# bo1929/krepp

Measured on AMD Instinct MI355X. Metric: reads/sec for `krepp dist` (150 bp), higher is better.
Workload: dtype u32/u64 integer + f64 likelihood; 1 GPU; 150bp reads vs 1000-genome synthetic index (Yule tree, -k 29 -w 35 -h 13, m4r1-frac, 2^25 rows), table inflated with random filler to 10 GB resident in HBM; index_inflated_in=a child process (handed over through /dev/shm), read_len=150, distinct_batches=2, lanes_per_batch=1, pipeline_streams=1, index_device_bytes=18867976828, hdist_th=4, parallelism=reads sharded x1, index replicated (RCCL bcast at load)

## Files before the change

### include/krepp_amd.h

```cpp
#ifndef KREPP_AMD_H
#define KREPP_AMD_H

#include <stddef.h>
#include <stdint.h>

#ifdef __cplusplus
extern "C" {
#endif

#define KR_API __attribute__((visibility("default")))

typedef enum kr_status {
  KR_OK = 0,
  KR_ERR_ARG = -1,
  KR_ERR_IO = -2,
  KR_ERR_FORMAT = -3,
  KR_ERR_NO_DEVICE = -4,
  KR_ERR_NOMEM = -5,
  KR_ERR_CAPACITY = -6,
  KR_ERR_STATE = -7,
  KR_ERR_UNSUPPORTED = -8
} kr_status;

#define KR_MAX_HDIST_TH 16u

typedef struct kr_host_index kr_host_index;

typedef struct kr_lib_view {
  const uint64_t* inc;
  const uint32_t* cmer;
  const uint32_t* pse;
  const double* rho;
  uint64_t nkmers;
  uint32_t nrows;
  uint32_t nsubsets;
  uint32_t nnodes;
  uint32_t r;
  uint32_t frac;
  uint32_t w;
} kr_lib_view;

typedef struct kr_index_view {
  uint32_t k, h, m;
  const uint8_t* ppos;
  const uint8_t* npos;
  uint32_t nlibs;
  const kr_lib_view* libs;
  uint32_t tree_nnodes;
  const uint8_t* node_kind;
  uint32_t wbackbone;
} kr_index_view;

KR_API int kr_host_index_load(const char* index_dir, kr_host_index** out);
KR_API int kr_host_sketch_load(const char* sketch_path, kr_host_index** out);
KR_API void kr_host_index_free(kr_host_index*);
KR_API int kr_host_index_view(const kr_host_index*, kr_index_view* out);
KR_API const char* kr_host_index_node_name(const kr_host_index*, uint32_t se);
KR_API const char* kr_host_index_node_label(const kr_host_index*, uint32_t se);
KR_API uint32_t kr_host_index_node_parent(const kr_host_index*, uint32_t se);
KR_API double kr_host_index_node_blen(const kr_host_index*, uint32_t se);

typedef struct kr_index kr_index;

#define KR_VIEW_HOST 0u
#define KR_VIEW_DEVICE 1u

KR_API int kr_index_upload(const kr_index_view* view, int device, uint32_t flags, kr_index** out);
KR_API void kr_index_free(kr_index*);

typedef struct kr_index_buffer {
  void* dptr;
  uint64_t bytes;
} kr_index_buffer;
KR_API int kr_index_export(const kr_index*, void* desc, uint64_t* desc_bytes, kr_index_buffer* bufs, uint32_t* nbufs);
KR_API int kr_index_import(const void* desc, uint64_t desc_bytes, int device, kr_index** out, kr_index_buffer* bufs,
                           uint32_t* nbufs);
KR_API uint64_t kr_index_device_bytes(const kr_index*);
KR_API uint32_t kr_index_slot_words(const kr_index*);
KR_API uint32_t kr_index_slot_format(const kr_index*);

KR_API int kr_index_broadcast(const kr_index* root, int ndev, const int* devices, kr_index** replicas);

typedef struct kr_params {
  uint32_t hdist_th;
  uint32_t tau;
  double chisq;
  double dist_max;
  uint32_t multi;
  uint32_t no_filter;
} kr_params;

KR_API void kr_params_default(kr_params*);

typedef struct kr_stream kr_stream;

KR_API int kr_stream_create(const kr_index*, const kr_params*, uint32_t max_reads, uint64_t max_bases,
                            uint64_t max_records, kr_stream** out);
KR_API void kr_stream_destroy(kr_stream*);

#define KR_BASES_HOST 0u
#define KR_BASES_DEVICE 1u
#define KR_TAP_ACCS 2u
#define KR_TAP_HITS 4u
#define KR_BASES_PINNED 8u
#define KR_ROWS_ONLY 16u
#define KR_ROWS_INDEXED 32u
#define KR_TILE_DEVICE 64u
#define KR_TILE_ROWS 128u

KR_API int kr_batch_submit(kr_stream*, const uint8_t* bases, const uint64_t* offsets, uint32_t nreads,
                           uint32_t flags);
KR_API int kr_batch_wait(kr_stream*);

typedef struct kr_result_view {
  uint32_t nreads;
  uint32_t nrecs;
  const uint32_t* read_off;
  const uint32_t* read_cnt;
  const uint32_t* read_onmers;
  const uint8_t* read_na;
  const uint32_t* rec_key;
  const uint8_t* rec_sel;
  const double* rec_d;
  const double* rec_v;
  const double* rec_chisq;
  const uint32_t* rec_hist;
  uint64_t rec_hist_stride;
  uint64_t nrows;
  const uint32_t* rec_dix;
  const double* dist_list;
  uint64_t ndist;
} kr_result_view;

KR_API int kr_batch_collect(kr_stream*, kr_result_view* out);
KR_API int kr_batch_collect_device(kr_stream*, kr_result_view* out);
KR_API int kr_debug_last_d2h_bytes(kr_stream*, uint64_t* bytes);
KR_API int kr_debug_place_fixed5(double v, char* out);

typedef struct kr_hit {
  uint32_t read;
  uint32_t kpos;
  uint32_t strand;
  uint32_t lib;
  uint64_t cmer_index;
  uint32_t hd;
  uint32_t se;
} kr_hit;
KR_API int kr_batch_hits(kr_stream*, const kr_hit** hits, uint64_t* nhits);
typedef struct kr_readtap {
  uint32_t hdist_filt[2];
} kr_readtap;
KR_API int kr_batch_readtaps(kr_stream*, const kr_readtap** taps);

KR_API int kr_debug_stream_move(kr_stream*, int which);
KR_API int kr_debug_stream_addrs(kr_stream*, uint64_t* out8);

KR_API int kr_debug_item_placement(kr_stream*, uint32_t* tried, uint32_t* kept, double* best_ns_per_read);

KR_API int kr_debug_front_end(const kr_index*, const uint8_t* bases, const uint64_t* offsets, uint32_t nreads,
                              uint32_t stride, uint32_t* rix, uint32_t* enc32, uint8_t* valid, uint8_t* pass);

KR_API int kr_debug_colour_classes(const uint32_t* pse_pairs , uint32_t nsubsets, const uint8_t* node_kind, uint32_t tree_nnodes,
                                   uint32_t* cls_out , uint32_t* pse_out , uint32_t* lists_out, uint64_t* nlist);

KR_API int kr_debug_brent(const kr_index*, uint32_t hdist_th, uint32_t n, const uint32_t* hist ,
                          const uint32_t* onmers, const double* rho, double* d_out, double* v_out);

KR_API int kr_debug_prefix(const uint32_t* values, uint32_t n, uint32_t block, uint32_t width, uint64_t* prefix , uint64_t* total);

KR_API int kr_llh_batch(const kr_index*, uint32_t hdist_th, uint32_t mode, uint64_t n, const double* hist, const double* uc,
                        const double* rho, const double* d_in, double* d_out, double* v_out);
KR_API int kr_llh_eval_indexed(const kr_index*, uint32_t th, uint64_t nprob, const double* hist, const double* uc, const double* rho,
                               uint64_t n, const uint32_t* pidx, const double* d_in, double* v_out);

typedef struct kr_timing {
  float ms_total;
  float ms_scan;
  float ms_acc;
  float ms_llh;
  float ms_h2d;
  uint32_t overflow_reads;
  uint32_t stack_spills;
  uint32_t lanes;
} kr_timing;
KR_API int kr_batch_timing(kr_stream*, kr_timing* out);

typedef struct kr_fastx kr_fastx;
typedef struct kr_fastx_batch {
  const uint8_t* bases;
  const uint64_t* offsets;
  const char* const* names;
  uint32_t nreads;
  uint32_t more;
} kr_fastx_batch;
KR_API int kr_fastx_open(const char* path, kr_fastx** out);
KR_API int kr_fastx_open_at(const char* path, uint64_t offset, kr_fastx** out);
KR_API int kr_fastx_next(kr_fastx*, uint64_t min_bases, kr_fastx_batch* out);
typedef struct kr_fastx_held kr_fastx_held;
KR_API int kr_fastx_detach(kr_fastx*, kr_fastx_held** out);
KR_API void kr_fastx_release(kr_fastx*, kr_fastx_held*);
KR_API uint64_t kr_fastx_parallel_chunks(const kr_fastx*);
KR_API void kr_fastx_pgz_stats(const kr_fastx*, uint64_t* parsed, uint64_t* discarded, uint64_t* gaps);
KR_API void kr_fastx_close(kr_fastx*);

KR_API int kr_format_dist(const kr_host_index*, const kr_result_view*, const char* const* names, char** text,
                          uint64_t* len);
KR_API int kr_format_seek(const kr_host_index*, const kr_index*, const kr_result_view*, uint32_t hdist_th,
                          const char* const* names, char** text, uint64_t* len);
KR_API int kr_stream_text_enable(kr_stream*, const kr_host_index*, uint64_t max_text_bytes, uint64_t max_id_bytes);
KR_API int kr_batch_submit_text(kr_stream*, const uint8_t* bases, const uint64_t* offsets, uint32_t nreads, uint32_t flags,
                                const char* ids, const uint32_t* id_off, uint32_t id_sep);
KR_API int kr_batch_collect_text(kr_stream*, const char** text, uint64_t* len);
KR_API uint32_t kr_debug_fixed5(double v, char* out);
KR_API void kr_free(void*);
KR_API void* kr_host_alloc(uint64_t bytes);
KR_API void kr_host_free(void*);

#define KR_FASTQ_OK 0u
#define KR_FASTQ_NOT_CLEAN 1u
#define KR_FASTQ_INCOMPLETE 2u
#define KR_FASTQ_LONG 3u
#define KR_FASTQ_CAPACITY 4u
typedef struct kr_fastq_parse {
  uint64_t consumed;
  uint64_t nbases;
  uint64_t id_bytes;
  uint64_t newlines;
  uint32_t nreads;
  uint32_t status;
  uint32_t rejected;
  uint32_t at_eof;
// ... 70 lines not shown
```

### krepp_amd/capi.py

```python
from __future__ import annotations

import ctypes as C
import os
from pathlib import Path

import numpy as np

_HERE = Path(__file__).resolve().parent
LIB_PATH = _HERE / "lib" / "libkrepp_amd.so"

KR_OK = 0
KR_ERR_ARG, KR_ERR_IO, KR_ERR_FORMAT, KR_ERR_NO_DEVICE = -1, -2, -3, -4
KR_ERR_NOMEM, KR_ERR_CAPACITY, KR_ERR_STATE, KR_ERR_UNSUPPORTED = -5, -6, -7, -8
KR_VIEW_HOST, KR_VIEW_DEVICE = 0, 1
KR_BASES_HOST, KR_BASES_DEVICE, KR_TAP_ACCS, KR_TAP_HITS, KR_BASES_PINNED, KR_ROWS_ONLY, KR_ROWS_INDEXED = 0, 1, 2, 4, 8, 16, 32
KR_TILE_DEVICE = 64
KR_TILE_ROWS = 128

u8p = C.POINTER(C.c_uint8)
u32p = C.POINTER(C.c_uint32)
u64p = C.POINTER(C.c_uint64)
f64p = C.POINTER(C.c_double)


class KrLibView(C.Structure):
    _fields_ = [("inc", u64p), ("cmer", u32p), ("pse", u32p), ("rho", f64p),
                ("nkmers", C.c_uint64), ("nrows", C.c_uint32), ("nsubsets", C.c_uint32),
                ("nnodes", C.c_uint32), ("r", C.c_uint32), ("frac", C.c_uint32), ("w", C.c_uint32)]


class KrIndexView(C.Structure):
    _fields_ = [("k", C.c_uint32), ("h", C.c_uint32), ("m", C.c_uint32),
                ("ppos", u8p), ("npos", u8p), ("nlibs", C.c_uint32), ("libs", C.POINTER(KrLibView)),
                ("tree_nnodes", C.c_uint32), ("node_kind", u8p), ("wbackbone", C.c_uint32)]


class KrIndexBuffer(C.Structure):
    _fields_ = [("dptr", C.c_void_p), ("bytes", C.c_uint64)]


class KrParams(C.Structure):
    _fields_ = [("hdist_th", C.c_uint32), ("tau", C.c_uint32), ("chisq", C.c_double),
                ("dist_max", C.c_double), ("multi", C.c_uint32), ("no_filter", C.c_uint32)]


class KrResultView(C.Structure):
    _fields_ = [("nreads", C.c_uint32), ("nrecs", C.c_uint32),
                ("read_off", u32p), ("read_cnt", u32p), ("read_onmers", u32p), ("read_na", u8p),
                ("rec_key", u32p), ("rec_sel", u8p), ("rec_d", f64p), ("rec_v", f64p),
                ("rec_chisq", f64p), ("rec_hist", u32p), ("rec_hist_stride", C.c_uint64), ("nrows", C.c_uint64),
                ("rec_dix", u32p), ("dist_list", f64p), ("ndist", C.c_uint64)]


class KrHit(C.Structure):
    _fields_ = [("read", C.c_uint32), ("kpos", C.c_uint32), ("strand", C.c_uint32), ("lib", C.c_uint32),
                ("cmer_index", C.c_uint64), ("hd", C.c_uint32), ("se", C.c_uint32)]


class KrTiming(C.Structure):
    _fields_ = [("ms_total", C.c_float), ("ms_scan", C.c_float), ("ms_acc", C.c_float), ("ms_llh", C.c_float),
                ("ms_h2d", C.c_float), ("overflow_reads", C.c_uint32), ("stack_spills", C.c_uint32), ("lanes", C.c_uint32)]


class KrFastxBatch(C.Structure):
    _fields_ = [("bases", u8p), ("offsets", u64p), ("names", C.POINTER(C.c_char_p)),
                ("nreads", C.c_uint32), ("more", C.c_uint32)]


KR_FASTQ_OK, KR_FASTQ_NOT_CLEAN, KR_FASTQ_INCOMPLETE, KR_FASTQ_LONG, KR_FASTQ_CAPACITY = 0, 1, 2, 3, 4


class KrFastqParse(C.Structure):
    _fields_ = [("consumed", C.c_uint64), ("nbases", C.c_uint64), ("id_bytes", C.c_uint64), ("newlines", C.c_uint64),
                ("nreads", C.c_uint32), ("status", C.c_uint32), ("rejected", C.c_uint32), ("at_eof", C.c_uint32),
                ("reserved", C.c_uint32 * 4)]


class KrMinimizerResult(C.Structure):
    _fields_ = [("keys", u64p), ("nkeys", C.c_uint64), ("n1", C.c_double), ("n2", C.c_double)]


class KrBuildParams(C.Structure):
    _fields_ = [("k", C.c_uint32), ("w", C.c_uint32), ("h", C.c_uint32), ("m", C.c_uint32), ("r", C.c_uint32),
                ("frac", C.c_uint32), ("num_threads", C.c_uint32), ("seed", C.c_uint32), ("ppos", u8p),
                ("gpu_minimizers", C.c_uint32), ("device", C.c_int32)]


EXPORTS = [
    "kr_host_index_load", "kr_host_sketch_load", "kr_format_seek", "kr_build_sketch", "kr_host_index_free", "kr_host_index_view", "kr_host_index_node_name",
    "kr_host_index_node_label", "kr_host_index_node_parent", "kr_host_index_node_blen",
    "kr_index_upload", "kr_index_free", "kr_index_export", "kr_index_import", "kr_index_device_bytes", "kr_index_slot_words", "kr_index_slot_format", "kr_index_broadcast",
    "kr_params_default", "kr_stream_create", "kr_stream_destroy", "kr_batch_submit", "kr_batch_wait",
    "kr_batch_collect", "kr_batch_collect_device", "kr_stream_text_enable", "kr_batch_submit_text", "kr_batch_collect_text",
    "kr_stream_fastq_enable", "kr_batch_submit_fastq", "kr_batch_fastq_names", "kr_debug_fastq_batch", "kr_debug_tile_layout", "kr_debug_tile_shape", "kr_batch_hits", "kr_batch_readtaps",
    "kr_debug_front_end", "kr_debug_stream_move", "kr_debug_stream_addrs", "kr_debug_item_placement", "kr_debug_brent", "kr_debug_prefix", "kr_debug_colour_classes", "kr_llh_batch", "kr_llh_eval_indexed", "kr_batch_timing",
    "kr_place_tree_create", "kr_place_tree_create_lineage", "kr_place_tree_nnodes", "kr_place_summary_add",
    "kr_place_summary_text", "kr_place_tree_free", "kr_place_tree_kinds", "kr_place_batch", "kr_place_stream", "kr_place_frame", "kr_place_counters",
    "kr_debug_last_d2h_bytes", "kr_debug_place_fixed5", "kr_place_text_counters", "kr_place_path_counters", "kr_fastx_open", "kr_fastx_open_at", "kr_fastx_next", "kr_fastx_detach", "kr_fastx_release", "kr_fastx_close", "kr_fastx_parallel_chunks", "kr_fastx_pgz_stats", "kr_format_dist", "kr_debug_fixed5", "kr_free", "kr_host_alloc", "kr_host_free",
    "kr_build_index", "kr_minimizers_cpu", "kr_minimizers_device", "kr_minimizers_free", "kr_last_error", "kr_version",
]

_lib = None


class KrError(RuntimeError):
    def __init__(self, code, msg):
        super().__init__(f"krepp_amd error {code}: {msg}")
        self.code = code


def load():
    global _lib
    if _lib is not None:
        return _lib
    if not LIB_PATH.exists():
        raise ImportError(f"{LIB_PATH} is missing: run `python -c 'import __graft_entry__ as g; g.build()'` "
                          "(the HIP extension is required; there is no CPU fallback)")
    lib = C.CDLL(str(LIB_PATH), mode=C.RTLD_GLOBAL)
    vp = C.c_void_p
    lib.kr_last_error.restype = C.c_char_p
    lib.kr_version.restype = C.c_char_p
    lib.kr_host_index_load.argtypes = [C.c_char_p, C.POINTER(vp)]
    lib.kr_host_index_free.argtypes = [vp]
    lib.kr_host_index_free.restype = None
    lib.kr_host_index_view.argtypes = [vp, C.POINTER(KrIndexView)]
    lib.kr_host_index_node_name.argtypes = [vp, C.c_uint32]
    lib.kr_host_index_node_name.restype = C.c_char_p
    lib.kr_host_index_node_label.argtypes = [vp, C.c_uint32]
    lib.kr_host_index_node_label.restype = C.c_char_p
    lib.kr_host_index_node_parent.argtypes = [vp, C.c_uint32]
    lib.kr_host_index_node_parent.restype = C.c_uint32
    lib.kr_host_index_node_blen.argtypes = [vp, C.c_uint32]
    lib.kr_host_index_node_blen.restype = C.c_double
    lib.kr_index_upload.argtypes = [C.POINTER(KrIndexView), C.c_int, C.c_uint32, C.POINTER(vp)]
    lib.kr_index_free.argtypes = [vp]
    lib.kr_index_free.restype = None
    lib.kr_index_export.argtypes = [vp, vp, u64p, C.POINTER(KrIndexBuffer), u32p]
    lib.kr_index_import.argtypes = [vp, C.c_uint64, C.c_int, C.POINTER(vp), C.POINTER(KrIndexBuffer), u32p]
    lib.kr_index_device_bytes.argtypes = [vp]
    lib.kr_index_broadcast.argtypes = [vp, C.c_int, C.POINTER(C.c_int), C.POINTER(vp)]
    lib.kr_index_device_bytes.restype = C.c_uint64
    lib.kr_index_slot_words.argtypes = [vp]
    lib.kr_index_slot_format.argtypes = [vp]
    lib.kr_index_slot_format.restype = C.c_uint32
    lib.kr_debug_stream_move.argtypes = [vp, C.c_int]
    lib.kr_debug_stream_addrs.argtypes = [vp, u64p]
    lib.kr_debug_item_placement.argtypes = [vp, u32p, u32p, C.POINTER(C.c_double)]
    lib.kr_index_slot_words.restype = C.c_uint32
    lib.kr_params_default.argtypes = [C.POINTER(KrParams)]
    lib.kr_params_default.restype = None
    lib.kr_stream_create.argtypes = [vp, C.POINTER(KrParams), C.c_uint32, C.c_uint64, C.c_uint64, C.POINTER(vp)]
    lib.kr_stream_destroy.argtypes = [vp]
    lib.kr_stream_destroy.restype = None
    lib.kr_batch_submit.argtypes = [vp, vp, vp, C.c_uint32, C.c_uint32]
    lib.kr_debug_fixed5.argtypes = [C.c_double, C.c_char_p]
    lib.kr_debug_fixed5.restype = C.c_uint32
    lib.kr_stream_text_enable.argtypes = [vp, vp, C.c_uint64, C.c_uint64]
    lib.kr_batch_submit_text.argtypes = [vp, vp, vp, C.c_uint32, C.c_uint32, vp, vp, C.c_uint32]
    lib.kr_batch_collect_text.argtypes = [vp, C.POINTER(vp), u64p]
    lib.kr_batch_wait.argtypes = [vp]
    lib.kr_batch_collect.argtypes = [vp, C.POINTER(KrResultView)]
    lib.kr_batch_collect_device.argtypes = [vp, C.POINTER(KrResultView)]
    lib.kr_batch_hits.argtypes = [vp, C.POINTER(C.POINTER(KrHit)), u64p]
    lib.kr_batch_readtaps.argtypes = [vp, C.POINTER(u32p)]
    lib.kr_debug_front_end.argtypes = [vp, vp, vp, C.c_uint32, C.c_uint32, vp, vp, vp, vp]
    lib.kr_debug_brent.argtypes = [vp, C.c_uint32, C.c_uint32, vp, vp, vp, vp, vp]
    lib.kr_debug_prefix.argtypes = [vp, C.c_uint32, C.c_uint32, C.c_uint32, vp, u64p]
    lib.kr_debug_colour_classes.argtypes = [vp, C.c_uint32, vp, C.c_uint32, vp, vp, vp, C.POINTER(C.c_uint64)]
    lib.kr_batch_timing.argtypes = [vp, C.POINTER(KrTiming)]
    lib.kr_llh_batch.argtypes = [vp, C.c_uint32, C.c_uint32, C.c_uint64, vp, vp, vp, vp, vp, vp]
    lib.kr_place_tree_create.argtypes = [vp, C.c_char_p, C.POINTER(vp)]
    lib.kr_place_tree_create_lineage.argtypes = [vp, C.c_char_p, C.POINTER(vp)]
    lib.kr_place_tree_nnodes.argtypes = [vp]
    lib.kr_place_tree_nnodes.restype = C.c_uint32
    lib.kr_place_summary_add.argtypes = [vp, vp, C.c_uint64, vp, C.POINTER(C.c_double)]
    lib.kr_place_summary_text.argtypes = [vp, vp, C.c_double, C.POINTER(vp), u64p]
    lib.kr_place_tree_free.argtypes = [vp]
    lib.kr_place_tree_free.restype = None
    lib.kr_place_tree_kinds.argtypes = [vp]
    lib.kr_place_tree_kinds.restype = u8p
    lib.kr_place_batch.argtypes = [vp, vp, vp, C.POINTER(KrResultView), vp, C.POINTER(C.c_char_p), C.POINTER(KrParams), C.c_int,
                                   C.POINTER(C.c_int), C.POINTER(vp), u64p, C.POINTER(vp), u64p]
    lib.kr_place_stream.argtypes = [vp, vp, vp, vp, C.c_uint32, vp, C.POINTER(C.c_char_p), C.POINTER(KrParams), C.c_int,
                                    C.POINTER(C.c_int), C.POINTER(vp), u64p, C.POINTER(vp), u64p]
    lib.kr_place_frame.argtypes = [vp, C.c_int, C.c_int, C.c_char_p, C.c_uint64, C.POINTER(vp), u64p]
    lib.kr_place_counters.argtypes = [u64p, u64p, u64p]
    lib.kr_place_counters.restype = None
    lib.kr_fastx_open.argtypes = [C.c_char_p, C.POINTER(vp)]
    lib.kr_fastx_open_at.argtypes = [C.c_char_p, C.c_uint64, C.POINTER(vp)]
    lib.kr_stream_fastq_enable.argtypes = [vp, C.c_uint64]
    lib.kr_batch_submit_fastq.argtypes = [vp, vp, C.c_uint64, C.c_uint32, C.c_uint32, C.POINTER(KrFastqParse)]
    lib.kr_batch_fastq_names.argtypes = [vp, C.POINTER(u64p), C.POINTER(u32p)]
    lib.kr_debug_fastq_batch.argtypes = [vp, vp, vp]
    lib.kr_debug_tile_layout.argtypes = [vp, u32p, u32p, vp, vp, vp, vp, vp]
    lib.kr_debug_tile_shape.argtypes = [C.c_uint64, C.c_uint32, u64p, u64p, u64p]
    lib.kr_fastx_next.argtypes = [vp, C.c_uint64, C.POINTER(KrFastxBatch)]
    lib.kr_fastx_detach.argtypes = [vp, C.POINTER(vp)]
    lib.kr_fastx_release.argtypes = [vp, vp]
    lib.kr_fastx_release.restype = None
    lib.kr_fastx_close.argtypes = [vp]
    lib.kr_fastx_close.restype = None
    lib.kr_format_dist.argtypes = [vp, C.POINTER(KrResultView), C.POINTER(C.c_char_p), C.POINTER(vp), u64p]
    lib.kr_free.argtypes = [vp]
    lib.kr_free.restype = None
    lib.kr_host_alloc.argtypes = [C.c_uint64]
    lib.kr_host_alloc.restype = vp
    lib.kr_host_free.argtypes = [vp]
    lib.kr_host_free.restype = None
    lib.kr_build_index.argtypes = [C.c_char_p, C.c_char_p, C.c_char_p, C.POINTER(KrBuildParams)]
    lib.kr_minimizers_cpu.argtypes = [C.POINTER(KrBuildParams), vp, vp, C.c_uint32, C.POINTER(KrMinimizerResult)]
    lib.kr_minimizers_device.argtypes = [C.c_int, C.POINTER(KrBuildParams), vp, vp, C.c_uint32, C.POINTER(KrMinimizerResult)]
    lib.kr_minimizers_free.argtypes = [C.POINTER(KrMinimizerResult)]
    lib.kr_minimizers_free.restype = None
    _lib = lib
    return lib


def check(rc):
    if rc != KR_OK:
        raise KrError(rc, load().kr_last_error().decode(errors="replace"))


def _np(ptr, n, dtype):
    if n == 0 or not ptr:
        return np.zeros(0, dtype=dtype)
    return np.ctypeslib.as_array(ptr, shape=(int(n),)).view(dtype).copy()

# ... 31 lines not shown
    def positions(self):
        return _np(self.view.ppos, self.view.h, np.uint8), _np(self.view.npos, self.view.k - self.view.h, np.uint8)

    def lib_arrays(self, i=0):
        lv = self.view.libs[i]
        return dict(inc=_np(lv.inc, lv.nrows, np.uint64), cmer=_np(lv.cmer, 2 * lv.nkmers, np.uint32).reshape(-1, 2),
                    pse=_np(lv.pse, 2 * lv.nsubsets, np.uint32).reshape(-1, 2), rho=_np(lv.rho, lv.nnodes, np.float64),
                    r=lv.r, frac=lv.frac, w=lv.w, nnodes=lv.nnodes, nsubsets=lv.nsubsets)

    def upload(self, device=0):
        return DeviceIndex.from_view(self.view, device, KR_VIEW_HOST, keep=self)

    def close(self):
        if self.h:
            self.lib.kr_host_index_free(self.h)
            self.h = C.c_void_p()

    def __del__(self):
        try:
            self.close()
        except Exception:
            pass


def default_params(**kw):
    p = KrParams()
    load().kr_params_default(C.byref(p))
    for k_, v in kw.items():
        setattr(p, k_, v)
    return p


class DeviceIndex:

    def __init__(self, handle, keep=None):
        self.lib = load()
        self.h = handle
        self._keep = keep

    @classmethod
    def from_view(cls, view, device=0, flags=KR_VIEW_HOST, keep=None):
        lib = load()
        h = C.c_void_p()
        check(lib.kr_index_upload(C.byref(view), int(device), int(flags), C.byref(h)))
        return cls(h, keep)

    def export(self):
        nb = C.c_uint64(0)
        n = C.c_uint32(0)
        check(self.lib.kr_index_export(self.h, None, C.byref(nb), None, C.byref(n)))
        desc = C.create_string_buffer(nb.value)
        bufs = (KrIndexBuffer * n.value)()
        check(self.lib.kr_index_export(self.h, desc, C.byref(nb), bufs, C.byref(n)))
        return desc.raw, [(b.dptr, b.bytes) for b in bufs]

    @classmethod
    def import_empty(cls, desc, device=0):
        lib = load()
        h = C.c_void_p()
        n = C.c_uint32(256)
        bufs = (KrIndexBuffer * 256)()
        check(lib.kr_index_import(desc, len(desc), int(device), C.byref(h), bufs, C.byref(n)))
        return cls(h), [(bufs[i].dptr, bufs[i].bytes) for i in range(n.value)]

    def broadcast(self, devices):
        n = len(devices)
        devs = (C.c_int * n)(*[int(d) for d in devices])
        outs = (C.c_void_p * n)()
        check(self.lib.kr_index_broadcast(self.h, n, devs, outs))
        return [DeviceIndex(C.c_void_p(outs[i])) for i in range(n)]

    @property
    def device_bytes(self):
        return int(self.lib.kr_index_device_bytes(self.h))

    @property
    def slot_words(self):
        return int(self.lib.kr_index_slot_words(self.h))

    @property
    def slot_format(self):
        return int(self.lib.kr_index_slot_format(self.h))

    def stream(self, params=None, max_reads=1 << 16, max_bases=None, max_records=0):
        return Stream(self, params or default_params(), max_reads, max_bases or max_reads * 160, max_records)

    def front_end(self, bases, offsets, stride):
        bases = np.ascontiguousarray(bases, dtype=np.uint8)
        offsets = np.ascontiguousarray(offsets, dtype=np.uint64)
        n = len(offsets) - 1
        rix = np.zeros((n, stride, 2), np.uint32)
        enc = np.zeros((n, stride, 2), np.uint32)
        valid = np.zeros((n, stride, 2), np.uint8)
        pas = np.zeros((n, stride, 2), np.uint8)
        check(self.lib.kr_debug_front_end(self.h, bases.ctypes.data, offsets.ctypes.data, n, stride,
                                          rix.ctypes.data, enc.ctypes.data, valid.ctypes.data, pas.ctypes.data))
        return rix, enc, valid, pas

    def brent(self, th, hist, onmers, rho):
        hist = np.ascontiguousarray(hist, dtype=np.uint32)
        onmers = np.ascontiguousarray(onmers, dtype=np.uint32)
        rho = np.ascontiguousarray(rho, dtype=np.float64)
        n = len(onmers)
        d = np.zeros(n)
        v = np.zeros(n)
        check(self.lib.kr_debug_brent(self.h, th, n, hist.ctypes.data, onmers.ctypes.data, rho.ctypes.data,
                                      d.ctypes.data, v.ctypes.data))
        return d, v

    def close(self):
        if self.h:
            self.lib.kr_index_free(self.h)
            self.h = C.c_void_p()

    def __del__(self):
        try:
            self.close()
        except Exception:
            pass


class Result:

    def __init__(self, rv, np_planes, copy_hist):
        n, c = rv.nreads, rv.nrecs
        self.nreads, self.nrecs, self.nrows = n, c, int(rv.nrows)
        self.read_off = _np(rv.read_off, n, np.uint32)
        self.read_cnt = _np(rv.read_cnt, n, np.uint32)
        self.read_onmers = _np(rv.read_onmers, n, np.uint32)
        self.read_na = _np(rv.read_na, n, np.uint8)
        key = _np(rv.rec_key, c, np.uint32)
        keep = key != 0
        self.rec_key = key[keep]
        self.rec_sel = _np(rv.rec_sel, c, np.uint8)[keep]
        if rv.rec_dix:
            self.rec_dix = _np(rv.rec_dix, c, np.uint32)[keep]
            self.dist_list = _np(rv.dist_list, int(rv.ndist), np.float64)
            self.rec_d = self.dist_list[self.rec_dix]
        else:
            self.rec_dix = None
            self.rec_d = _np(rv.rec_d, c, np.float64)[keep]
        self.rec_v = _np(rv.rec_v, c, np.float64)[keep] if rv.rec_v else None
        self.rec_chisq = _np(rv.rec_chisq, c, np.float64)[keep] if rv.rec_chisq else None
        self.rec_hist = (_np(rv.rec_hist, c * np_planes, np.uint32).reshape(np_planes, -1).T[keep]
                         if copy_hist and rv.rec_hist and c else (np.zeros((0, np_planes), np.uint32) if copy_hist else None))
        rr = np.zeros(c, np.uint32)
        nzr = np.nonzero(self.read_cnt)[0]
        if c and len(nzr):
            start = np.zeros(c, np.int64)
            start[self.read_off[nzr]] = self.read_off[nzr].astype(np.int64) + 1
            at = np.zeros(c + 1, np.uint32)
            at[self.read_off[nzr].astype(np.int64) + 1] = nzr
            rr = at[np.maximum.accumulate(start)]
        self.rec_read = rr[keep]
        newpos = np.cumsum(keep) - 1
        nz = self.read_cnt > 0
        self.read_off = np.where(nz, newpos[np.minimum(self.read_off, max(c - 1, 0))] if c else 0, 0).astype(np.uint32)
        self.nrecs = int(keep.sum())

    def rows(self):
        sel = self.rec_sel.astype(bool)
        return sorted(zip(self.rec_read[sel].tolist(), (self.rec_key[sel] >> 1).tolist(), self.rec_d[sel].tolist()))


class Stream:
    def __init__(self, dindex, params, max_reads, max_bases, max_records=0):
        self.lib = load()
        self.ix = dindex
        self.params = params
        self.h = C.c_void_p()
        check(self.lib.kr_stream_create(dindex.h, C.byref(params), int(max_reads), int(max_bases), int(max_records), C.byref(self.h)))
        self._keep = None
        self._flags = 0

    def submit(self, bases, offsets, flags=0):
        bases = np.ascontiguousarray(bases, dtype=np.uint8)
        offsets = np.ascontiguousarray(offsets, dtype=np.uint64)
        self._keep = (bases, offsets)
        self._flags = flags
        check(self.lib.kr_batch_submit(self.h, bases.ctypes.data, offsets.ctypes.data, len(offsets) - 1, flags))

    def submit_device(self, bases_ptr, offsets_ptr, nreads, flags=0):
        self._flags = flags | KR_BASES_DEVICE
        check(self.lib.kr_batch_submit(self.h, int(bases_ptr), int(offsets_ptr), int(nreads), self._flags))

    def wait(self):
        check(self.lib.kr_batch_wait(self.h))

    def collect(self):
        rv = KrResultView()
        check(self.lib.kr_batch_collect(self.h, C.byref(rv)))
        self._rv = rv
        return Result(rv, self.params.hdist_th + 1, bool(self._flags & KR_TAP_ACCS))

    def collect_view(self):
        rv = KrResultView()
        check(self.lib.kr_batch_collect(self.h, C.byref(rv)))
        self._rv = rv
        return rv

    def last_d2h_bytes(self):
        b = C.c_uint64(0)
        self.lib.kr_debug_last_d2h_bytes.argtypes = [C.c_void_p, C.POINTER(C.c_uint64)]
        check(self.lib.kr_debug_last_d2h_bytes(self.h, C.byref(b)))
        return int(b.value)

    def collect_device(self):
        rv = KrResultView()
        check(self.lib.kr_batch_collect_device(self.h, C.byref(rv)))
        return rv

    def hits(self):
        p = C.POINTER(KrHit)()
        n = C.c_uint64()
        check(self.lib.kr_batch_hits(self.h, C.byref(p), C.byref(n)))
        dt = np.dtype([("read", "<u4"), ("kpos", "<u4"), ("strand", "<u4"), ("lib", "<u4"), ("cmer_index", "<u8"),
                       ("hd", "<u4"), ("se", "<u4")])
        if n.value == 0:
            return np.zeros(0, dt)
        raw = C.string_at(p, n.value * C.sizeof(KrHit))
        return np.frombuffer(raw, dtype=dt).copy()

    def readtaps(self, nreads):
        p = u32p()
        check(self.lib.kr_batch_readtaps(self.h, C.byref(p)))
        return _np(p, 2 * nreads, np.uint32).reshape(-1, 2)

    def debug_move(self, which):
        check(self.lib.kr_debug_stream_move(self.h, which))

    def item_placement(self):
        a, b, c = C.c_uint32(0), C.c_uint32(0), C.c_double(0)
        check(self.lib.kr_debug_item_placement(self.h, C.byref(a), C.byref(b), C.byref(c)))
        return {"tried": a.value, "kept": b.value, "scan_ns_per_read": c.value}

    def debug_addrs(self):
        a = (C.c_uint64 * 8)()
        check(self.lib.kr_debug_stream_addrs(self.h, a))
        return dict(zip(("items", "counters", "cursors", "rd_off", "rd_it_off", "rd_filt", "rec_key", "dd"), [int(x) for x in a]))

    def timing(self):
        t = KrTiming()
        check(self.lib.kr_batch_timing(self.h, C.byref(t)))
        return t

    def format_seek(self, host_index, device_index, names, hdist_th=4):
        arr = (C.c_char_p * len(names))(*[n.encode() for n in names])
        txt = C.c_void_p()
        ln = C.c_uint64()
        self.lib.kr_format_seek.argtypes = [C.c_void_p, C.c_void_p, C.POINTER(KrResultView), C.c_uint32, C.POINTER(C.c_char_p),
                                            C.POINTER(C.c_void_p), C.POINTER(C.c_uint64)]
        check(self.lib.kr_format_seek(host_index.h, device_index.h, C.byref(self._rv), hdist_th, arr, C.byref(txt), C.byref(ln)))
        s = C.string_at(txt, ln.value).decode()
        self.lib.kr_free(txt)
        return s

    def text_enable(self, host_index, max_text_bytes, max_id_bytes):
        check(self.lib.kr_stream_text_enable(self.h, host_index.h, int(max_text_bytes), int(max_id_bytes)))
        self._text_on = True

    def submit_text(self, bases, offsets, names, flags=0, sep=1):
        bases = np.ascontiguousarray(bases, dtype=np.uint8)
        offsets = np.ascontiguousarray(offsets, dtype=np.uint64)
        enc = [n.encode() for n in names]
        blob = (b"\0" * sep).join(enc) + b"\0" * sep
        lens = np.fromiter((len(e) + sep for e in enc), dtype=np.uint32, count=len(enc))
        id_off = np.zeros(len(enc) + 1, dtype=np.uint32)
        np.cumsum(lens, out=id_off[1:])
        ids = np.frombuffer(blob, dtype=np.uint8)
        self._keep = (bases, offsets, ids, id_off)
        self._flags = flags | KR_ROWS_ONLY
        check(self.lib.kr_batch_submit_text(self.h, bases.ctypes.data, offsets.ctypes.data, len(offsets) - 1, flags, ids.ctypes.data, id_off.ctypes.data, sep))

    def submit_text_device(self, bases_ptr, offsets_ptr, nreads, names, flags=0, sep=1):
        enc = [n.encode() for n in names]
        ids = np.frombuffer((b"\0" * sep).join(enc) + b"\0" * sep, dtype=np.uint8)
        id_off = np.zeros(len(enc) + 1, dtype=np.uint32)
        np.cumsum(np.fromiter((len(e) + sep for e in enc), dtype=np.uint32, count=len(enc)), out=id_off[1:])
        self._keep = (ids, id_off)
        self._flags = flags | KR_BASES_DEVICE | KR_ROWS_ONLY
        check(self.lib.kr_batch_submit_text(self.h, int(bases_ptr), int(offsets_ptr), int(nreads), flags | KR_BASES_DEVICE, ids.ctypes.data, id_off.ctypes.data, sep))

    def fastq_enable(self, max_raw_bytes):
        check(self.lib.kr_stream_fastq_enable(self.h, int(max_raw_bytes)))

    def submit_fastq(self, raw, flags=0, at_eof=1):
        raw = bytes(raw)
        n = len(raw)
        if getattr(self, "_pinned_cap", 0) < max(n, 1):
            if getattr(self, "_pinned", None):
                self.lib.kr_host_free(self._pinned)
            self._pinned = self.lib.kr_host_alloc(max(n, 1))
            if not self._pinned:
                raise MemoryError("kr_host_alloc failed")
            self._pinned_cap = max(n, 1)
        C.memmove(self._pinned, raw, n)
        self._raw = raw
        out = KrFastqParse()
        check(self.lib.kr_batch_submit_fastq(self.h, self._pinned, n, flags, at_eof, C.byref(out)))
        self._fq_nreads = out.nreads
        text = getattr(self, "_text_on", False) and not (flags & (KR_TAP_ACCS | KR_TAP_HITS))
        self._flags = flags | KR_BASES_DEVICE | (KR_ROWS_ONLY if text else 0)
        return {f: getattr(out, f) for f in ("consumed", "nbases", "id_bytes", "newlines", "nreads", "status", "rejected", "at_eof")}

    def fastq_names(self):
        pos, ln = u64p(), u32p()
        check(self.lib.kr_batch_fastq_names(self.h, C.byref(pos), C.byref(ln)))
        n = self._fq_nreads
        if n == 0:
            return []
        p = np.ctypeslib.as_array(pos, shape=(n,))
        q = np.ctypeslib.as_array(ln, shape=(n,))
        return [self._raw[int(a):int(a) + int(b)].decode("latin-1") for a, b in zip(p, q)]

    def fastq_batch(self, summary):
        offs = np.zeros(summary["nreads"] + 1, np.uint64)
        bases = np.zeros(max(1, summary["nbases"]), np.uint8)
        check(self.lib.kr_debug_fastq_batch(self.h, bases.ctypes.data, offs.ctypes.data))
        return [bases[int(offs[i]):int(offs[i + 1])].tobytes() for i in range(summary["nreads"])]

    def tile_layout(self, nreads):
        nv, nl = C.c_uint32(0), C.c_uint32(0)
        check(self.lib.kr_debug_tile_layout(self.h, C.byref(nv), C.byref(nl), None, None, None, None, None))
        out = {"nv": int(nv.value), "nlong": int(nl.value)}
        if out["nv"] == 0:
            return out
        voff, vtile = np.zeros(out["nv"] + 1, np.uint64), np.zeros(out["nv"], np.uint8)
        rfirst, longs = np.zeros(nreads, np.uint32), np.zeros(2 * out["nlong"], np.uint32)
        check(self.lib.kr_debug_tile_layout(self.h, C.byref(nv), C.byref(nl), voff.ctypes.data, vtile.ctypes.data, rfirst.ctypes.data,
                                            longs.ctypes.data, None))
        bases = np.zeros(max(1, int(voff[-1])), np.uint8)
        check(self.lib.kr_debug_tile_layout(self.h, C.byref(nv), C.byref(nl), None, None, None, None, bases.ctypes.data))
        out.update(voff=voff, vtile=vtile, rfirst=rfirst, longs=longs.reshape(-1, 2), bases=bases[:int(voff[-1])])
        return out

    def collect_text(self):
        txt = C.c_void_p()
        ln = C.c_uint64()
        check(self.lib.kr_batch_collect_text(self.h, C.byref(txt), C.byref(ln)))
        return C.string_at(txt, ln.value) if ln.value else b""

    def format_dist(self, host_index, names):
        arr = (C.c_char_p * len(names))(*[n.encode() for n in names])
        txt = C.c_void_p()
        ln = C.c_uint64()
        check(self.lib.kr_format_dist(host_index.h, C.byref(self._rv), arr, C.byref(txt), C.byref(ln)))
        s = C.string_at(txt, ln.value).decode()
        self.lib.kr_free(txt)
        return s

    def close(self):
        if self.h:
            self.lib.kr_stream_destroy(self.h)
            self.h = C.c_void_p()
        if getattr(self, "_pinned", None):
            self.lib.kr_host_free(self._pinned)
            self._pinned, self._pinned_cap = None, 0

    def __del__(self):
        try:
            self.close()
        except Exception:
            pass


def tile_shape(length, k):
    a, b, c = C.c_uint64(0), C.c_uint64(0), C.c_uint64(0)
    check(load().kr_debug_tile_shape(int(length), int(k), C.byref(a), C.byref(b), C.byref(c)))
    return int(a.value), int(b.value), int(c.value)


def debug_prefix(values, block, width):
    values = np.ascontiguousarray(values, dtype=np.uint32)
    prefix = np.zeros(len(values), np.uint64)
    total = C.c_uint64(0)
    check(load().kr_debug_prefix(values.ctypes.data, len(values), block, width, prefix.ctypes.data, C.byref(total)))
    return prefix, total.value


def colour_classes(pse, node_kind):
    lib = load()
    pse = np.ascontiguousarray(pse, dtype=np.uint32).reshape(-1, 2)
    node_kind = np.ascontiguousarray(node_kind, dtype=np.uint8)
    n = len(pse)
    cls = np.zeros(n, np.uint32)
    out = np.zeros((n, 2), np.uint32)
    nl = C.c_uint64(0)
    rc = lib.kr_debug_colour_classes(pse.ctypes.data, n, node_kind.ctypes.data, len(node_kind) - 1, cls.ctypes.data, out.ctypes.data, None,
                                     C.byref(nl))
    lists = np.zeros(max(1, nl.value), np.uint32)
    if rc != 0:
        check(lib.kr_debug_colour_classes(pse.ctypes.data, n, node_kind.ctypes.data, len(node_kind) - 1, cls.ctypes.data, out.ctypes.data,
                                          lists.ctypes.data, C.byref(nl)))
    return cls, out, lists[: nl.value]


def read_fastx(path, min_bases=76800, stats=None, detach=0, offset=None):
    lib = load()
    lib.kr_fastx_parallel_chunks.restype = C.c_uint64
    lib.kr_fastx_parallel_chunks.argtypes = [C.c_void_p]
    h = C.c_void_p()
    if offset is None:
        check(lib.kr_fastx_open(os.fsencode(str(path)), C.byref(h)))
    else:
        check(lib.kr_fastx_open_at(os.fsencode(str(path)), int(offset), C.byref(h)))
    names, chunks, lens = [], [], []

    def take(b):
        if b.nreads:
            offs = np.ctypeslib.as_array(b.offsets, shape=(b.nreads + 1,)).copy()
            chunks.append(np.ctypeslib.as_array(b.bases, shape=(int(offs[-1]),)).copy() if offs[-1] else np.zeros(0, np.uint8))
            lens.extend(np.diff(offs).tolist())
            names.extend(b.names[i].decode() for i in range(b.nreads))

    held = []
    try:
        while True:
            b = KrFastxBatch()
            check(lib.kr_fastx_next(h, min_bases, C.byref(b)))
            if detach:
                hp = C.c_void_p()
                check(lib.kr_fastx_detach(h, C.byref(hp)))
                held.append((b, hp))
                while len(held) > detach:
                    ob, ohp = held.pop(0)
                    take(ob)
                    lib.kr_fastx_release(h, ohp)
            else:
                take(b)
            if not b.more:
                break
        for ob, ohp in held:
            take(ob)
            lib.kr_fastx_release(h, ohp)
    finally:
        if stats is not None:
            stats["parallel_chunks"] = int(lib.kr_fastx_parallel_chunks(h))
            a, b_, c_ = C.c_uint64(0), C.c_uint64(0), C.c_uint64(0)
            lib.kr_fastx_pgz_stats.restype = None
            lib.kr_fastx_pgz_stats.argtypes = [C.c_void_p, C.POINTER(C.c_uint64), C.POINTER(C.c_uint64), C.POINTER(C.c_uint64)]
            lib.kr_fastx_pgz_stats(h, C.byref(a), C.byref(b_), C.byref(c_))
            stats["gzip_chunks"] = {"parsed": int(a.value), "discarded": int(b_.value), "gaps": int(c_.value)}
        lib.kr_fastx_close(h)
    bases = np.concatenate(chunks) if chunks else np.zeros(0, np.uint8)
    offsets = np.zeros(len(lens) + 1, np.uint64)
    offsets[1:] = np.cumsum(np.asarray(lens, dtype=np.uint64))
    return names, bases, offsets


def place_counters():
    a, b = C.c_uint64(0), C.c_uint64(0)
    load().kr_place_counters(C.byref(a), C.byref(b), None)
    return int(a.value), int(b.value)


def place_text_counters():
    a, b = C.c_uint64(0), C.c_uint64(0)
    load().kr_place_text_counters.restype = None
    load().kr_place_text_counters(C.byref(a), C.byref(b))
    return int(a.value), int(b.value)
# ... 145 lines not shown
```

### krepp_amd/csrc/kr_common.h

```cpp
#ifndef KR_COMMON_H
#define KR_COMMON_H

#include "krepp_amd.h"

#include <atomic>
#include <cmath>
#include <cstdio>
#include <functional>
#include <string>
#include <vector>

namespace kr {

int fail(int code, const std::string& msg);
void clear_error();

struct TreeNode {
  std::string label;
  double blen;
  uint32_t parent;
  uint8_t kind;
};

struct HostTree {
  std::vector<TreeNode> nodes;
  uint32_t nnodes() const { return (uint32_t)nodes.size() - 1; }
  std::string name(uint32_t se) const;
};

bool parse_newick(const std::string& text, HostTree& out, std::string& err);
void balanced_tree(const std::vector<std::string>& names, HostTree& out);

void parallel_for(int n, const std::function<void(int)>& f);
int parallel_width();
unsigned usable_cpus();

uint64_t leaf_name_hash(const std::string& name);
uint64_t rehash64(uint64_t sh);

struct BuildCfg {
  uint32_t k, w, h, m, r;
  bool frac;
};
struct LshPositions {
  uint32_t k = 0, h = 0;
  std::vector<uint8_t> ppos, npos;
  std::vector<uint8_t> pasc;
  uint32_t rix(uint64_t bp) const;
  uint32_t enc32(uint64_t bp) const;
};
bool make_positions(uint32_t k, uint32_t h, const uint8_t* ppos, LshPositions& out);
double hll12_estimate(const uint8_t* reg);
inline int64_t build_row(uint32_t rix, const BuildCfg& c)
{
  uint32_t res = rix % c.m;
  if (c.frac ? res <= c.r : res == c.r) return c.frac ? (int64_t)(rix / c.m) * (c.r + 1) + res : (int64_t)(rix / c.m);
  return -1;
}
#if defined(__HIPCC__)
#define KR_HD __host__ __device__
#else
#define KR_HD
#endif
KR_HD inline bool fixed5_exact(double v, uint32_t* n_out)
{
  if (!(v >= 0.0 && v < 1000.0)) return false;
  const double sc = v * 100000.0;
  const double err = fma(v, 100000.0, -sc);
  const double fl = floor(sc), fr = sc - fl;
  uint32_t n = (uint32_t)fl;
  const double t = fr - 0.5;
  if (t > 0.0 || (t == 0.0 && (err > 0.0 || (err == 0.0 && (n & 1u))))) ++n;
  if (n >= 100000000u) return false;
  *n_out = n;
  return true;
}
KR_HD inline uint32_t fixed5_digits(uint32_t n, char* out)
{
  uint32_t ip = n / 100000u, fp = n - ip * 100000u;
  char tmp[4];
  uint32_t k = 0, o = 0;
  do {
    tmp[k++] = (char)('0' + ip % 10u);
    ip /= 10u;
  } while (ip);
  while (k) out[o++] = tmp[--k];
  out[o++] = '.';
  for (int q = 4; q >= 0; --q) {
    out[o + (uint32_t)q] = (char)('0' + fp % 10u);
    fp /= 10u;
  }
  return o + 5u;
}
inline size_t fmt_fixed5(double v, char* out)
{
  const bool neg = std::signbit(v);
  const double d = neg ? -v : v;
  if (d >= 0.0 && d < 1000.0) {
    const double sc = d * 100000.0, fl = std::floor(sc), fr = sc - fl;
    if (std::fabs(fr - 0.5) > 1e-6) {
      const uint64_t n = (uint64_t)fl + (fr > 0.5 ? 1u : 0u);
      uint64_t ip = n / 100000u, fp = n % 100000u;
      char tmp[8];
      size_t k = 0, o = 0;
      if (neg) out[o++] = '-';
      do {
        tmp[k++] = (char)('0' + ip % 10u);
        ip /= 10u;
      } while (ip);
      while (k) out[o++] = tmp[--k];
      out[o++] = '.';
      for (int q = 4; q >= 0; --q) {
        out[o + q] = (char)('0' + fp % 10u);
        fp /= 10u;
      }
      return o + 5;
    }
  }
  return (size_t)snprintf(out, 64, "%.5f", v);
}

inline uint64_t fmix64(uint64_t v)
{
  v ^= v >> 33;
  v *= 0xff51afd7ed558ccdull;
  v ^= v >> 33;
  v *= 0xc4ceb9fe1a85ec53ull;
  v ^= v >> 33;
  return v;
}
void extract_contig_cpu(const uint8_t* seq, uint64_t len, const BuildCfg& c, const LshPositions& lsh,
                        std::vector<uint64_t>& keys, double& n1, double& n2);
bool contig_end_special(const uint8_t* seq, uint64_t len, const BuildCfg& c, uint64_t& x, uint64_t& z);

struct PlaceTreeArrays {
  uint32_t pn = 0, nidx = 0;
  const uint32_t* parent = nullptr;
  const uint32_t* eff = nullptr;
  const uint8_t* elig = nullptr;
  const uint32_t* lo = nullptr;
  const uint32_t* idx_to_pt = nullptr;
  const uint32_t* depth = nullptr;
  const double* blen = nullptr;
  const uint32_t* card = nullptr;
  const char* labels = nullptr;
  const uint32_t* label_off = nullptr;
};
struct PlaceDeviceResult {
  uint32_t nreads = 0;
  const uint32_t* rd_c0 = nullptr;
  const uint32_t* rd_info = nullptr;
  const uint32_t* c_se = nullptr;
  const double *c_d = nullptr, *c_v = nullptr, *c_chisq = nullptr;
  uint64_t kept = 0;
  bool overflow = false;
  uint32_t heavy_reads = 0;
  const char* text = nullptr;
  uint64_t text_len = 0;
  uint64_t text_flags = 0;
};
}
struct kr_stream;
namespace kr {
int place_on_device(kr_stream* s, const void* tree_tag, const PlaceTreeArrays& T, const uint32_t* read_len, uint32_t tau,
                    bool no_filter, double chisq, PlaceDeviceResult* out);
int place_device_begin(kr_stream* s, const void* tree_tag, const PlaceTreeArrays& T, const uint32_t* read_len);
int place_device_launch(kr_stream* s, const PlaceTreeArrays& T, uint32_t r0, uint32_t n, uint32_t tau, bool no_filter, double chisq);
int place_device_finish(kr_stream* s, const PlaceTreeArrays& T, uint32_t r0, uint32_t n, uint32_t tau, bool no_filter, double chisq,
                        uint64_t kept_base, PlaceDeviceResult* out);
uint32_t place_stream_nreads(const kr_stream* s);
void* big_alloc(size_t n);
void big_free(void* p);
void place_device_abort(kr_stream* s);
int place_device_text_begin(kr_stream* s, const PlaceTreeArrays& T, const char* const* names, uint32_t nreads, int tabular, bool multi);
enum PlacePath : uint32_t {
  kPathRerunCand = 0, kPathRerunKeep, kPathListCut, kPathGivenUp, kPathText1, kPathText2, kPathText4, kPathText8, kPathText16, kPathRanges,
  kPathLastCnt0, kPathLastCnt3, kPathLastCnt12, kPathLastText, kPathLastCandCap, kPathLastKeepCap, kPathLastTextCap, kPathLastFlags,
  kPathLastTextFlags, kPathLastAttempts, kPathCount
};
extern std::atomic<uint64_t> g_place_paths[kPathCount];

}

#endif
```

### krepp_amd/csrc/kr_dev_common.inc

```

constexpr int kWave = 64;
constexpr int kSegPos = 128;
constexpr int kPlaneWords = kSegPos / 32;
constexpr int kMaxLibs = 16;
constexpr int kStackCap = 256;
constexpr int kLeanStack = 192;
__host__ __device__ inline uint32_t lean_stack_bytes(uint32_t bm_words) { uint32_t b = 5u * bm_words; b = (b + 15u) & ~15u; return b > kLeanStack * 8u ? b : kLeanStack * 8u; }
constexpr int kLdsSlots = 64;
#ifndef KR_ACC_LEAN_WPE
#define KR_ACC_LEAN_WPE 6
#endif
#ifndef KR_ACC_PIPE
#define KR_ACC_PIPE 1
#endif
#ifndef KR_ACC_LEAN_EV_WORDS
#define KR_ACC_LEAN_EV_WORDS 1216
#endif
#ifndef KR_ACC_LEAN2_EV_HALVES
#define KR_ACC_LEAN2_EV_HALVES 4
#endif
__host__ __device__ inline uint32_t lean_ev_words(uint32_t np, uint32_t segs = 1)
{
  const uint32_t w = KR_ACC_LEAN_EV_WORDS ? (uint32_t)KR_ACC_LEAN_EV_WORDS : (uint32_t)kLdsSlots * np * 5u ;
  return segs == 1 ? w : (w * (uint32_t)KR_ACC_LEAN2_EV_HALVES / 2u + 3u) & ~3u;
}
constexpr int kLdsProbeMax = 8;
constexpr int kMaxPlanes = KR_MAX_HDIST_TH + 1;
constexpr int kHistWords = (kMaxPlanes + 3) / 4;

constexpr uint32_t kSlotFilter = 9u;
__host__ __device__ inline uint32_t slot_words(uint32_t code) { return code == 0 ? 0u : (code == 8 ? 48u : (code == kSlotFilter ? 64u : 1u << code)); }

constexpr uint32_t kFiltLineCodes = 40u, kFiltSlotCodes = 80u;
constexpr uint32_t kFiltMaxTh = 6u;
__host__ __device__ inline uint32_t filt_code24(uint32_t enc) { return (enc & 0xFFFu) | ((enc >> 4) & 0xFFF000u); }
__host__ __device__ inline uint32_t filt_rest8(uint32_t enc) { return ((enc >> 12) & 0xFu) | ((enc >> 24) & 0xF0u); }

struct DevLib {
  const uint64_t* bkt;
  const uint32_t* enc;
  const uint32_t* se;
  const uint2* pse;
  const double* rho;
  const uint32_t* slots;
  const uint32_t* occ;
  const uint32_t* leaflist;
  const uint2* sx;
  uint64_t nkmers, nlist;
  uint32_t nrows, nsubsets, nnodes, numer;
  uint32_t slot_log2w;
};

struct DevIndex {
  uint32_t k, h, m, nlibs, tree_nnodes;
  uint32_t m_shift;
  PextMask pmask, nmask;
  const uint4* fe_tab;
  uint64_t ppk[2], npk[2];
  uint32_t nleaves;
  const uint32_t* node_info;
  const uint32_t* leaf_se;
  const int32_t* res_lib;
  const DevLib* libs;
  uint64_t res_mask;
  DevLib lib0;
};

struct LlhConst {
  uint32_t k, h, th, dbg;
  double binom_k[32];
  double binom_hnk[kMaxPlanes];
};

struct DevParams {
  uint32_t th, np;
  uint32_t multi, no_filter, dmax_set;
  uint32_t dbg;
  double chisq, dist_max;
};

enum CounterSlot : uint32_t {
  kCtRecSlots = 0,
  kCtErr = 1,
  kCtL2Reads = 2,
  kCtTapHits = 3,
  kCtRecords = 4,
  kCtLlhCursor = 5,
  kCtItemSlots = 6,
  kCtStEvents = 9,
  kCtStKeys = 10,
  kCtStBatches = 11,
  kCtStBig = 12,
  kCtStLevelTiles = 13,
  kCtStMaxKeys = 14,
  kCtStMaxEvents = 15,
  kCtCycLevel = 16,
  kCtCycFinalize = 17,
  kCtCycRead = 18,
  kCtProblems = 22,
  kCtLongReads = 25,
  kCtStackSpills = 26,
  kCtRows = 27,
  kCtTileHoles = 28,
  kCtCount = 29
};
constexpr uint32_t kCounterWords = (kCtCount + 31u) & ~31u;
enum CursorSet : uint32_t { kCurScan = 0, kCurAcc1 = 1 , kCurAccMerge = 2 , kCurAcc2 = 3 , kCurSets = 4 };

struct BatchOut {
  uint32_t* counters;
  uint32_t* cursors;
  uint32_t* rd_off;
  uint32_t* rd_cnt;
  uint32_t* rd_onmers;
  uint32_t* rd_filt;
  uint8_t* rd_na;
  uint32_t* rec_read;
  uint32_t* rec_key;
  uint32_t* rec_hist;
  double* rec_d;
  double* rec_v;
  double* rec_chisq;
  uint8_t* rec_sel;
  uint64_t* rec_w0;
  uint32_t hist_always;
  uint32_t keep_v;
  uint32_t* rec_rep;
  uint32_t* rep_list;
  double2* rep_dv;
  uint32_t rep_cap;
  ulonglong2* dd_table;
  uint32_t* dd_direct;
  double2* dd_dv;
  uint32_t* dd_ohist;
  uint8_t* dd_oslot;
  const uint8_t* dd_cls;
  uint32_t dd_nodes;
  uint32_t dd_slots;
  uint32_t dd_shift;
  uint32_t rec_cap;
  uint64_t rec_stride;
  kr_hit* hits;
  uint32_t hit_cap;
  uint2* items;
  const uint8_t* v_tile;
  uint32_t rows_mode;
  uint32_t* rd_rcnt;
  uint32_t* rd_roff;
  uint32_t* row_bsum;
  uint32_t* row_key;
  double* row_d;
  uint32_t rows_indexed;
  uint32_t* row_dix;
  double* dist_list;
  uint32_t item_cap;
  uint32_t* rd_it_off;
  uint32_t* rd_it_cnt;
  uint32_t rec_chunk;
  uint32_t* long_list;
  uint32_t* g_planes;
  uint32_t* g_counts;
  uint32_t* g_list;
  uint64_t* stk_spill;
  uint32_t nslots2;
  uint32_t g_list_words;
  uint32_t ev_spill, tab_spill, kt_spill;
  uint32_t bm_words;
};

enum : uint32_t { kErrRecCap = 1u, kErrStack = 2u, kErrTable = 4u, kErrHitCap = 8u, kErrItemCap = 16u };

// ... 298 lines not shown
```

### krepp_amd/csrc/kr_dev_likelihood.inc

```

struct LlhProblem {
  double mc[kMaxPlanes];
  double uc, rho;
};

struct DD {
  double hi, lo;
};
__device__ __forceinline__ DD dd_mul(DD a, DD b)
{
  double p = a.hi * b.hi;
  double e = fma(a.hi, b.hi, -p);
  e = fma(a.hi, b.lo, e);
  e = fma(a.lo, b.hi, e);
  double s = p + e;
  return DD{s, e - (s - p)};
}
__device__ __forceinline__ double pown_dd(double x, uint32_t n)
{
  DD r{1.0, 0.0}, b{x, 0.0};
  while (n) {
    if (n & 1u) r = dd_mul(r, b);
    n >>= 1;
    if (n) b = dd_mul(b, b);
// ... 1126 lines not shown
      tot += c[q];
    }
    uint32_t run = out.row_bsum[b] + block_scan_excl(tot);
#pragma unroll
    for (uint32_t q = 0; q < 4; ++q) {
      s_off[q0 + q] = run;
      if (rb + q0 + q < nreads) out.rd_roff[rb + q0 + q] = run;
      run += c[q];
    }
    __syncthreads();
    constexpr uint32_t U = 4;
    for (uint32_t qa = w; qa < kRowBlock && rb + qa < nreads; qa += 4u * U) {
      uint32_t o[U], n[U], ky[U], xr[U];
      double xd[U];
      uint8_t sl[U];
#pragma unroll
      for (uint32_t u = 0; u < U; ++u) {
        const uint32_t q = qa + 4u * u;
        const bool there = q < kRowBlock && rb + q < nreads;
        o[u] = there ? out.rd_off[rb + q] : 0u, n[u] = there ? out.rd_cnt[rb + q] : 0u;
      }
#pragma unroll
      for (uint32_t u = 0; u < U; ++u) {
        const bool on = lane < n[u];
        sl[u] = on ? out.rec_sel[o[u] + lane] : (uint8_t)0;
        ky[u] = on ? out.rec_key[o[u] + lane] : 0u;
        xr[u] = 0u, xd[u] = 0.0;
        if (INDEXED)
          xr[u] = on ? out.rec_rep[o[u] + lane] : 0u;
        else
          xd[u] = on ? out.rec_d[o[u] + lane] : 0.0;
      }
#pragma unroll
      for (uint32_t u = 0; u < U; ++u) {
        const uint32_t q = qa + 4u * u;
        if (n[u] == 0) continue;
        uint32_t pos = s_off[q];
        {
          const bool sel = sl[u] != 0;
          const uint64_t sm = __ballot(sel);
          if (sel) {
            const uint32_t at = pos + (uint32_t)__popcll(sm & lt);
            out.row_key[at] = ky[u];
            if (INDEXED)
              out.row_dix[at] = xr[u];
            else
              out.row_d[at] = xd[u];
          }
          pos += (uint32_t)__popcll(sm);
        }
        for (uint32_t i0 = 64u; i0 < n[u]; i0 += 64u) {
          const uint32_t i = i0 + lane;
          const bool sel = i < n[u] && out.rec_sel[o[u] + i] != 0;
          const uint64_t sm = __ballot(sel);
          if (sel) {
            const uint32_t at = pos + (uint32_t)__popcll(sm & lt);
            out.row_key[at] = out.rec_key[o[u] + i];
            if (INDEXED)
              out.row_dix[at] = out.rec_rep[o[u] + i];
            else
              out.row_d[at] = out.rec_d[o[u] + i];
          }
          pos += (uint32_t)__popcll(sm);
        }
      }
    }
    __syncthreads();
  }
}

__global__ void kr_build_occ(const uint64_t* bkt, uint32_t nrows, uint32_t* occ)
{
  const uint32_t nw = (nrows + 31u) / 32u;
  for (uint32_t w = blockIdx.x * blockDim.x + threadIdx.x; w < nw; w += gridDim.x * blockDim.x) {
    uint32_t bits = 0;
    for (uint32_t j = 0; j < 32u; ++j) {
      const uint32_t r = w * 32u + j;
      if (r < nrows && (bkt[r] & 0xFFFFFFull) != 0) bits |= 1u << j;
    }
    occ[w] = bits;
  }
}

__global__ void kr_build_slots(const uint64_t* bkt, const uint32_t* enc, uint32_t nrows, uint32_t words, uint32_t* slots)
{
  const uint64_t n = (uint64_t)nrows * words;
  for (uint64_t i = blockIdx.x * (uint64_t)blockDim.x + threadIdx.x; i < n; i += (uint64_t)gridDim.x * blockDim.x) {
    const uint32_t row = (uint32_t)(i / words), wd = (uint32_t)(i - (uint64_t)row * words);
    const uint64_t b = bkt[row];
    const uint64_t st = b >> 24;
    const uint32_t ln = (uint32_t)(b & 0xFFFFFFu);
    uint32_t x = 0xFFFFFFFFu;
    if (wd == 0)
      x = ln;
    else if (wd == 1)
      x = (uint32_t)st;
    else if (wd - 2u < ln)
      x = enc[st + wd - 2u];
    slots[i] = x;
  }
}
```

### krepp_amd/csrc/kr_dev_scan.inc

```

constexpr int kListCap = 128;
struct ProbeList {
  lds_u64* bkt;
  lds_u32* q;
  lds_u32* tag;
};

struct Cand {
  uint64_t b0, b1;
  uint32_t q0, q1;
  uint32_t lib0, lib1;
};

template <bool SL, bool SLOT>
__device__ __forceinline__ Cand fetch_group_fe(const DevIndex& ix, const FrontEnd& fe, uint32_t& nvalid)
{
  Cand c;
  nvalid = __popcll(__ballot(fe.valid));
  int lib = -1;
  c.b0 = 0, c.b1 = 0, c.lib0 = 0, c.lib1 = 0;
  c.q0 = fe.enc32[0];
  c.q1 = fe.enc32[1];
  const uint32_t* d0 = nullptr;
  const uint32_t* d1 = nullptr;
// ... 64 lines not shown
  uint32_t rd_start;
  uint32_t err;
  uint32_t filt0, filt1;
  uint32_t cur_seg;
  uint32_t n_st;
  lds_u64* stage;
};
constexpr uint32_t kItemStage = 256;
#ifndef KR_ITEM_CHUNK
#define KR_ITEM_CHUNK 2048
#endif
constexpr uint32_t kItemChunk = KR_ITEM_CHUNK;
#ifndef KR_SCAN_READ_CHUNK
#define KR_SCAN_READ_CHUNK 32
#endif
constexpr uint32_t kReadChunk = KR_SCAN_READ_CHUNK;
constexpr uint32_t kCursors = 32, kCursorStride = 32;
struct ReadCursor {
  uint32_t* cur;
  uint32_t nreads, range, c, tried, chunk;
  __device__ __forceinline__ void init(uint32_t* base, uint32_t n, uint32_t home, uint32_t reads_per_visit = kReadChunk)
  {
    cur = base, nreads = n, range = (n + kCursors - 1) / kCursors, c = home % kCursors, tried = n ? 0 : kCursors, chunk = reads_per_visit;
  }
  __device__ __forceinline__ bool next(uint32_t& r0, uint32_t& r1)
  {
    while (tried < kCursors) {
      const uint32_t lo = c * range, hi = min(lo + range, nreads);
      uint32_t o = 0;
      if (lane_id() == 0) o = atomicAdd(&cur[c * kCursorStride], chunk);
      o = __shfl(o, 0);
      if (lo + o < hi) {
        r0 = lo + o, r1 = min(r0 + chunk, hi);
        return true;
      }
      c = (c + 1) % kCursors, ++tried;
    }
    return false;
  }
};

__device__ __forceinline__ bool item_reserve(const BatchOut& out, ScanWave& sw, uint32_t n)
{
  if (sw.it_next + n <= sw.it_end) return true;
  const uint32_t have = sw.it_next - sw.rd_start;
  const uint32_t size = (have + n + kItemChunk + 15u) & ~15u;
  uint32_t base = 0;
  if (lane_id() == 0) base = atomicAdd(&out.counters[kCtItemSlots], size);
  base = __shfl(base, 0);
  if ((uint64_t)base + size > out.item_cap) {
    sw.err |= kErrItemCap;
    return false;
  }
  if (have) {
    __builtin_amdgcn_fence(__ATOMIC_ACQ_REL, "workgroup");
    for (uint32_t i = lane_id(); i < have; i += 64) {
      const uint32_t* src = reinterpret_cast<const uint32_t*>(out.items + sw.rd_start + i);
      out.items[base + i] = make_uint2(gload(src), gload(src + 1));
    }
  }
  sw.rd_start = base;
  sw.it_next = base + have;
  sw.it_end = base + size;
  return true;
}

__device__ __forceinline__ void flush_stage(const BatchOut& out, ScanWave& sw)
{
  if (sw.n_st == 0) return;
  WAVE_SYNC();
  const uint32_t n16 = (sw.n_st + 15u) & ~15u;
  if (item_reserve(out, sw, n16)) {
    for (uint32_t i = lane_id(); i < n16; i += 64) {
      const uint64_t v = i < sw.n_st ? sw.stage[i] : 0ull;
      out.items[sw.it_next + i] = make_uint2((uint32_t)v, (uint32_t)(v >> 32));
    }
    sw.it_next += sw.n_st;
  }
  sw.n_st = 0;
  WAVE_SYNC();
}

constexpr uint32_t kItemMarker = 0x80000000u;
template <bool SL, bool TAP, bool FK = false>
__device__ __forceinline__ void emit_hits(const DevIndex& ix, const BatchOut& out, ScanWave& sw, uint32_t read, uint32_t base0,
                                          uint32_t tg, uint64_t e_al, uint32_t c, uint32_t pend, uint32_t hds)
{
  const uint64_t lt = (1ull << lane_id()) - 1ull;
  const uint32_t seg = base0 >> 7;
  while (__ballot(pend != 0) != 0) {
    const bool has = pend != 0;
    const uint32_t e = has ? (uint32_t)__ffs((int)pend) - 1u : 0u;
    const uint32_t hd = (hds >> (8u * e)) & 31u;
    const uint64_t idx = e_al + 4ull * c + e;
    if (has) {
      if (tag_strand(tg))
        sw.filt1 = min(sw.filt1, hd);
      else
        sw.filt0 = min(sw.filt0, hd);
      if (TAP) {
        const uint32_t se = get_lib<SL>(ix, tag_lib(tg)).se[idx];
        const uint32_t hix = atomicAdd(&out.counters[kCtTapHits], 1u);
        if (hix < out.hit_cap) {
          kr_hit h;
          h.read = read;
          h.kpos = base0 + tag_pos(tg);
          h.strand = tag_strand(tg);
          h.lib = tag_lib(tg);
          h.cmer_index = idx;
          h.hd = hd;
          h.se = (se >> 30) == 1u ? ix.leaf_se[se & kColMask] : (se & kColMask);
          out.hits[hix] = h;
        } else {
          atomicOr(&out.counters[kCtErr], kErrHitCap);
        }
      }
    }
    const uint64_t hm = __ballot(has);
    const uint32_t mark = seg != sw.cur_seg ? 1u : 0u;
    if (sw.n_st + (uint32_t)__popcll(hm) + mark > kItemStage) flush_stage(out, sw);
    if (mark && lane_id() == 0) sw.stage[sw.n_st] = (uint64_t)seg | ((uint64_t)kItemMarker << 32);
    sw.n_st += mark;
    sw.cur_seg = seg;
    if (has)
      sw.stage[sw.n_st + __popcll(hm & lt)] =
        (uint64_t)(uint32_t)idx | ((uint64_t)(FK ? ((tg & 0xFFFu) | (7u << 12) | (hd << 15) | ((uint32_t)(idx >> 32) << 23))
                                                 : ((tg & 0xFFFu) | (hd << 12) | ((uint32_t)(idx >> 32) << 17))) << 32);
    sw.n_st += (uint32_t)__popcll(hm);
    pend &= pend - 1u;
  }
}

template <int LOG_G, int CPL, bool SL, bool TAP>
__device__ __forceinline__ void scan_group(const DevIndex& ix, const DevParams& P, const BatchOut& out, ScanWave& sw,
                                           const ProbeList& pl, lds_u32* queue, lds_u32* stepinfo, uint32_t nact, uint32_t read,
                                           uint32_t base0)
{
  constexpr uint32_t G = 1u << LOG_G, PPS = 64u >> LOG_G;
  constexpr uint32_t kBits = 64u / CPL * CPL;
  const uint32_t lane = lane_id(), sub = lane & (G - 1u);
  uint32_t p0 = 0, cb = 0;
  while (p0 < nact) {
    uint64_t hitbits = 0;
    uint32_t step = 0;
    while (p0 < nact && step < kBits) {
      const uint32_t pi = p0 + (lane >> LOG_G);
      const bool on = pi < nact;
      const uint64_t b = on ? pl.bkt[pi] : 0ull;
      const uint32_t q = on ? pl.q[pi] : 0u;
      const uint64_t st = b >> 24;
      const uint32_t tot = (uint32_t)(st & 3u) + (uint32_t)(b & 0xFFFFFFu);
      const uint32_t nch = on ? (tot + 3u) >> 2 : 0u;
      const uint32_t* enc = get_lib<SL>(ix, SL ? 0u : tag_lib(pl.tag[on ? pi : 0u])).enc + (st & ~3ull);
      for (; step < kBits && __ballot(sub + cb * G < nch) != 0; cb += CPL, step += CPL) {
        if (lane < (uint32_t)CPL) stepinfo[step + lane] = p0 | (((cb + lane) * G) << 8);
        uint4 v[CPL];
#pragma unroll
        for (int j = 0; j < CPL; ++j) {
          const uint32_t c = sub + (cb + (uint32_t)j) * G;
          v[j] = make_uint4(0, 0, 0, 0);
          if (c < nch) v[j] = *reinterpret_cast<const uint4*>(enc + 4u * c);
        }
        uint32_t r = 0;
#pragma unroll
        for (int j = 0; j < CPL; ++j) {
          const uint32_t m = min(min(hd_lr32(v[j].x, q), hd_lr32(v[j].y, q)), min(hd_lr32(v[j].z, q), hd_lr32(v[j].w, q)));
          r |= (m <= P.th && sub + (cb + (uint32_t)j) * G < nch) ? (1u << j) : 0u;
        }
        hitbits |= (uint64_t)r << step;
      }
      if (__ballot(sub + cb * G < nch) == 0) p0 += PPS, cb = 0;
    }
    if (P.dbg & 1u) hitbits = 0;
    const uint32_t cnt = (uint32_t)__popcll(hitbits);
    uint32_t inc = cnt;
#pragma unroll
    for (int d = 1; d < 64; d <<= 1) {
      const uint32_t o = __shfl_up(inc, d);
      if (lane >= (uint32_t)d) inc += o;
    }
    const uint32_t H = __shfl(inc, 63);
    uint64_t hb = hitbits;
    uint32_t slot = inc - cnt;
    WAVE_SYNC();
    for (uint32_t w0 = 0; w0 < H; w0 += 64) {
      while (__ballot(hb != 0 && slot < w0 + 64u) != 0) {
        if (hb != 0 && slot < w0 + 64u) {
          const uint32_t si = stepinfo[(uint32_t)__ffsll((long long)hb) - 1u];
          queue[slot - w0] = ((si & 255u) + (lane >> LOG_G)) | ((sub + (si >> 8)) << 8);
          hb &= hb - 1;
          ++slot;
        }
      }
      WAVE_SYNC();
      uint32_t pend = 0, hds = 0, tg = 0, c = 0;
      uint64_t e_al = 0;
      if (lane < min(64u, H - w0)) {
        const uint32_t d = queue[lane], probe = d & 255u;
        c = d >> 8;
        const uint64_t b = pl.bkt[probe];
// ... 3 lines not shown
        e_al = st & ~3ull;
        const int rel0 = (int)(st & 3u), tot = rel0 + (int)(uint32_t)(b & 0xFFFFFFu);
        const uint4 v = *reinterpret_cast<const uint4*>(get_lib<SL>(ix, tag_lib(tg)).enc + e_al + 4u * c);
        pend = chunk_hits(v, rel0 - 4 * (int)c, tot - 4 * (int)c, q, P.th, hds);
      }
      WAVE_SYNC();
      emit_hits<SL, TAP>(ix, out, sw, read, base0, tg, e_al, c, pend, hds);
    }
  }
}

template <int LOG_G, int CPL, bool SL, bool TAP>
__device__ __forceinline__ void scan_group_slots(const DevIndex& ix, const DevParams& P, const BatchOut& out, ScanWave& sw,
                                                 const ProbeList& pl, lds_u32* queue, uint32_t nact, uint32_t read, uint32_t base0)
{
  constexpr uint32_t G = 1u << LOG_G, PPS = 64u >> LOG_G, W = G * CPL * 4u, CAP = W - 2u;
  static_assert((kListCap / PPS) * CPL <= 64, "one hit bit per (pass, chunk)");
  const uint32_t lane = lane_id(), sub = lane & (G - 1u);
  uint64_t hitbits = 0;
  uint32_t step = 0;
  for (uint32_t p0 = 0; p0 < nact; p0 += PPS, step += CPL) {
    const uint32_t pi = p0 + (lane >> LOG_G);
    const bool on = pi < nact;
    const uint32_t row = on ? (uint32_t)pl.bkt[pi] : 0u;
    const uint32_t q = on ? pl.q[pi] : 0u;
    const DevLib L = get_lib<SL>(ix, SL ? 0u : tag_lib(pl.tag[on ? pi : 0u]));
    const uint32_t* slot = L.slots + (uint64_t)row * W;
    uint4 v[CPL];
#pragma unroll
    for (int j = 0; j < CPL; ++j) {
      v[j] = make_uint4(0, 0, 0, 0);
      if (on) v[j] = *reinterpret_cast<const uint4*>(slot + 4u * (sub + (uint32_t)j * G));
    }
    uint32_t r = 0;
#pragma unroll
    for (int j = 0; j < CPL; ++j) {
      const uint32_t m = min(min(hd_lr32(v[j].x, q), hd_lr32(v[j].y, q)), min(hd_lr32(v[j].z, q), hd_lr32(v[j].w, q)));
      r |= (m <= P.th && on) ? (1u << j) : 0u;
    }
    hitbits |= (uint64_t)r << step;
    if (__ballot(on && sub == 0 && v[0].x > CAP) != 0) {
      const uint32_t blen = __shfl(v[0].x, lane & ~(G - 1u)), bstart = __shfl(v[0].y, lane & ~(G - 1u));
      const bool lg = on && blen > CAP;
      const uint64_t st = (uint64_t)bstart + CAP;
      const uint64_t e_al = st & ~3ull;
      const int rel0 = (int)(st & 3u), tot = rel0 + (lg ? (int)(blen - CAP) : 0);
      const uint32_t nch = lg ? (uint32_t)(tot + 3) >> 2 : 0u;
      const uint32_t tg = pl.tag[on ? pi : 0u];
      for (uint32_t c = sub; __ballot(c < nch) != 0; c += G) {
        uint32_t pend = 0, hds = 0;
        if (c < nch) {
          const uint4 w = *reinterpret_cast<const uint4*>(L.enc + e_al + 4u * c);
          pend = chunk_hits(w, rel0 - 4 * (int)c, tot - 4 * (int)c, q, P.th, hds);
        }
        if (P.dbg & 1u) pend = 0;
        emit_hits<SL, TAP>(ix, out, sw, read, base0, tg, e_al, c, pend, hds);
      }
    }
  }
  if (P.dbg & 1u) hitbits = 0;
  const uint32_t cnt = (uint32_t)__popcll(hitbits);
  uint32_t inc = cnt;
#pragma unroll
  for (int d = 1; d < 64; d <<= 1) {
    const uint32_t o = __shfl_up(inc, d);
    if (lane >= (uint32_t)d) inc += o;
  }
  const uint32_t H = __shfl(inc, 63);
  uint64_t hb = hitbits;
  uint32_t slot_i = inc - cnt;
  for (uint32_t w0 = 0; w0 < H; w0 += 64) {
    while (__ballot(hb != 0 && slot_i < w0 + 64u) != 0) {
      if (hb != 0 && slot_i < w0 + 64u) {
        const uint32_t bit = (uint32_t)__ffsll((long long)hb) - 1u;
        const uint32_t pass = bit / (uint32_t)CPL, j = bit - pass * (uint32_t)CPL;
        queue[slot_i - w0] = (pass * PPS + (lane >> LOG_G)) | ((sub + j * G) << 8);
        hb &= hb - 1;
        ++slot_i;
      }
    }
    WAVE_SYNC();
    uint32_t pend = 0, hds = 0, tg = 0, c = 0;
    uint64_t e_al = 0;
    if (lane < min(64u, H - w0)) {
      const uint32_t d = queue[lane], probe = d & 255u;
      c = d >> 8;
      const uint32_t row = (uint32_t)pl.bkt[probe];
      const uint32_t q = pl.q[probe];
      tg = pl.tag[probe];
      const uint32_t* slot = get_lib<SL>(ix, tag_lib(tg)).slots + (uint64_t)row * W;
      const uint2 hdr = *reinterpret_cast<const uint2*>(slot);
      const uint4 v = *reinterpret_cast<const uint4*>(slot + 4u * c);
      const int nin = (int)min(hdr.x, CAP);
      pend = chunk_hits(v, 2 - 4 * (int)c, nin + 2 - 4 * (int)c, q, P.th, hds);
      e_al = (uint64_t)hdr.y - 2ull;
    }
    WAVE_SYNC();
    emit_hits<SL, TAP>(ix, out, sw, read, base0, tg, e_al, c, pend, hds);
  }
}

template <int LOG_G, int CPL, bool SL, bool TAP, bool SLOT>
__device__ __forceinline__ void scan_read(const DevIndex& ix, const DevParams& P, const BatchIn& in, const BatchOut& out,
                                          uint32_t read, ScanWave& sw, const ProbeList& pl, lds_u32* queue, lds_u32* stepinfo, lds_u32* meta)
{
  const uint32_t lane = lane_id();
  const uint64_t lt = (1ull << lane) - 1ull;
  const uint64_t off0 = in.offsets[read], off1 = in.offsets[read + 1];
  const uint8_t* seq = in.bases + off0;
  const uint64_t len = off1 - off0;
  const uint32_t k = ix.k;
  const uint64_t nkm = len >= k ? len - k + 1 : 0;
  uint32_t onmers = 0;
  sw.it_next = min((sw.it_next + 15u) & ~15u, sw.it_end);
  sw.rd_start = sw.it_next;
  sw.n_st = 0;
  sw.cur_seg = 0;
  sw.filt0 = 0xFFFFFFFFu, sw.filt1 = 0xFFFFFFFFu;
  for (uint64_t base0 = 0; base0 < nkm; base0 += kSegPos) {
    const uint32_t npos_seg = (uint32_t)min((uint64_t)kSegPos, nkm - base0);
    SegBits sb;
    load_segment(seq, len, base0, sb);
#pragma unroll
    for (int pp = 0; pp < 2; ++pp) {
      if (pp == 1 && npos_seg <= 64) break;
      uint32_t nv = 0;
      const Cand cur = fetch_group<SL, SLOT>(ix, sb, pp, npos_seg, nv);
      onmers += nv;
      const bool a0 = SLOT ? cur.b0 != 0 : (cur.b0 & 0xFFFFFFu) != 0, a1 = SLOT ? cur.b1 != 0 : (cur.b1 & 0xFFFFFFu) != 0;
      const uint64_t m0 = __ballot(a0), m1 = __ballot(a1);
      const uint32_t n0 = __popcll(m0), nact = n0 + __popcll(m1);
      if (a0) {
        const uint32_t i = __popcll(m0 & lt);
        pl.bkt[i] = cur.b0;
        pl.q[i] = cur.q0;
        pl.tag[i] = (64u * pp + lane) | (cur.lib0 << 8);
      }
      if (a1) {
        const uint32_t i = n0 + __popcll(m1 & lt);
        pl.bkt[i] = cur.b1;
        pl.q[i] = cur.q1;
        pl.tag[i] = (64u * pp + lane) | (1u << 7) | (cur.lib1 << 8);
      }
      WAVE_SYNC();
      if (!(P.dbg & 4u)) {
        if (SLOT)
          scan_group_slots<LOG_G, CPL, SL, TAP>(ix, P, out, sw, pl, queue, nact, read, (uint32_t)base0);
        else
          scan_group<LOG_G, CPL, SL, TAP>(ix, P, out, sw, pl, queue, stepinfo, nact, read, (uint32_t)base0);
      }
      WAVE_SYNC();
    }
  }
  flush_stage(out, sw);
  uint32_t f0 = sw.filt0, f1 = sw.filt1;
#pragma unroll
  for (int d = 32; d >= 1; d >>= 1) {
    f0 = min(f0, (uint32_t)__shfl_xor(f0, d));
    f1 = min(f1, (uint32_t)__shfl_xor(f1, d));
  }
  if (lane == 0) {
    meta[0 * kReadChunk] = sw.rd_start;
    meta[1 * kReadChunk] = sw.it_next - sw.rd_start;
    meta[2 * kReadChunk] = onmers;
    meta[3 * kReadChunk] = f0;
    meta[4 * kReadChunk] = f1;
  }
}

#ifndef KR_SCAN_WPE
#define KR_SCAN_WPE 6
#endif
#ifndef KR_SCAN_WPE_SLOT
#define KR_SCAN_WPE_SLOT 4
#endif
constexpr int kScanWaves = 4;
template <int LOG_G, int CPL, bool SL, bool TAP, bool SLOT>
__global__ __launch_bounds__(kScanWaves* kWave, (SLOT ? KR_SCAN_WPE_SLOT : KR_SCAN_WPE)) void kr_scan_kernel_t(DevIndex ix, DevParams P, BatchIn in, BatchOut out)
{
  __shared__ __attribute__((aligned(16))) uint64_t s_bkt[kScanWaves][kListCap];
  __shared__ uint32_t s_q[kScanWaves][kListCap], s_tag[kScanWaves][kListCap], s_queue[kScanWaves][64], s_step[kScanWaves][64];
// ... 34 lines not shown
```

### krepp_amd/csrc/kr_dev_scan_pipe.inc

```

#ifndef KR_SCAN_DEPTH
#define KR_SCAN_DEPTH 1
#endif
#ifndef KR_SCAN_PIPE_WPE
#define KR_SCAN_PIPE_WPE 4
#endif
#ifndef KR_SCAN_PIPE_FE
#define KR_SCAN_PIPE_FE 2
#endif

struct SlotList {
  lds_u32* row;
  lds_u32* q;
  lds_u32* tag;
};
struct GroupDesc {
  uint32_t nact, read, base0, slot;
  bool last;
};

struct SegRaw {
  uint32_t c[3];
};
__device__ __forceinline__ SegRaw segment_request(const uint8_t* seq, uint64_t len, uint64_t base0)
// ... 124 lines not shown
#pragma unroll
  for (int d = 0; d < DEPTH; ++d) {
    const uint32_t pi = (c * DEPTH + (uint32_t)d) * PPS + (lane >> LOG_G);
    const bool on = pi < nact;
    const uint32_t row = on ? L.row[pi] : 0u;
    const uint32_t* slot = get_lib<SL>(ix, SL ? 0u : tag_lib(L.tag[on ? pi : 0u])).slots + (uint64_t)row * W;
#pragma unroll
    for (int j = 0; j < CPL; ++j) {
      v[d * CPL + j] = make_uint4(0, 0, 0, 0);
      if (on) v[d * CPL + j] = *reinterpret_cast<const uint4*>(slot + 4u * (sub + (uint32_t)j * G));
    }
  }
}

template <int LOG_G, int CPL, int DEPTH, bool SL, bool TAP>
__device__ __forceinline__ uint64_t pipe_test(const DevIndex& ix, const DevParams& P, const BatchOut& out, ScanWave& sw, const SlotList& L,
                                              const GroupDesc& g, uint32_t c, const uint4 (&v)[DEPTH * CPL])
{
  constexpr uint32_t G = 1u << LOG_G, PPS = 64u >> LOG_G, W = G * CPL * 4u, CAP = W - 2u;
  const uint32_t lane = lane_id(), sub = lane & (G - 1u);
  uint64_t bits = 0;
#pragma unroll
  for (int d = 0; d < DEPTH; ++d) {
    const uint32_t p = c * DEPTH + (uint32_t)d;
    const uint32_t pi = p * PPS + (lane >> LOG_G);
    const bool on = pi < g.nact;
    const uint32_t q = on ? L.q[pi] : 0u;
    uint32_t r = 0;
#pragma unroll
    for (int j = 0; j < CPL; ++j) {
      const uint4 w = v[d * CPL + j];
      const uint32_t m = min(min(hd_lr32(w.x, q), hd_lr32(w.y, q)), min(hd_lr32(w.z, q), hd_lr32(w.w, q)));
      r |= (m <= P.th && on) ? (1u << j) : 0u;
    }
    bits |= (uint64_t)r << (p * CPL);
    const uint32_t blen0 = v[d * CPL].x;
    if (__ballot(on && sub == 0 && blen0 > CAP) != 0) {
      const uint32_t blen = __shfl(blen0, lane & ~(G - 1u)), bstart = __shfl(v[d * CPL].y, lane & ~(G - 1u));
      const bool lg = on && blen > CAP;
      const uint64_t st = (uint64_t)bstart + CAP;
      const uint64_t e_al = st & ~3ull;
      const int rel0 = (int)(st & 3u), tot = rel0 + (lg ? (int)(blen - CAP) : 0);
      const uint32_t nch = lg ? (uint32_t)(tot + 3) >> 2 : 0u;
      const uint32_t tg = L.tag[on ? pi : 0u];
      const DevLib Lb = get_lib<SL>(ix, SL ? 0u : tag_lib(tg));
      for (uint32_t cc = sub; __ballot(cc < nch) != 0; cc += G) {
        uint32_t pend = 0, hds = 0;
        if (cc < nch) {
          const uint4 w = *reinterpret_cast<const uint4*>(Lb.enc + e_al + 4u * cc);
          pend = chunk_hits(w, rel0 - 4 * (int)cc, tot - 4 * (int)cc, q, P.th, hds);
        }
        if (P.dbg & 1u) pend = 0;
        emit_hits<SL, TAP>(ix, out, sw, g.read, g.base0, tg, e_al, cc, pend, hds);
      }
    }
  }
  return (P.dbg & 1u) ? 0ull : bits;
}

template <int LOG_G, int CPL, bool SL, bool TAP>
__device__ __forceinline__ void pipe_resolve(const DevIndex& ix, const DevParams& P, const BatchOut& out, ScanWave& sw, const SlotList& L,
                                             lds_u32* queue, const GroupDesc& g, uint64_t hitbits)
{
  constexpr uint32_t G = 1u << LOG_G, PPS = 64u >> LOG_G, W = G * CPL * 4u, CAP = W - 2u;
  const uint32_t lane = lane_id(), sub = lane & (G - 1u);
  const uint32_t cnt = (uint32_t)__popcll(hitbits);
  const uint32_t inc = wave_scan_incl(cnt);
  const uint32_t H = (uint32_t)__builtin_amdgcn_readlane((int)inc, 63);
  uint64_t hb = hitbits;
  uint32_t slot_i = inc - cnt;
  for (uint32_t w0 = 0; w0 < H; w0 += 64) {
    while (__ballot(hb != 0 && slot_i < w0 + 64u) != 0) {
      if (hb != 0 && slot_i < w0 + 64u) {
        const uint32_t bit = (uint32_t)__ffsll((long long)hb) - 1u;
        const uint32_t pass = bit / (uint32_t)CPL, j = bit - pass * (uint32_t)CPL;
        queue[slot_i - w0] = (pass * PPS + (lane >> LOG_G)) | ((sub + j * G) << 8);
        hb &= hb - 1;
        ++slot_i;
      }
    }
    WAVE_SYNC();
    uint32_t pend = 0, hds = 0, tg = 0, c = 0;
    uint64_t e_al = 0;
    if (lane < min(64u, H - w0)) {
      const uint32_t d = queue[lane], probe = d & 255u;
      c = d >> 8;
      const uint32_t row = L.row[probe];
      const uint32_t q = L.q[probe];
      tg = L.tag[probe];
      const uint32_t* slot = get_lib<SL>(ix, tag_lib(tg)).slots + (uint64_t)row * W;
      const uint2 hdr = *reinterpret_cast<const uint2*>(slot);
      const uint4 v = *reinterpret_cast<const uint4*>(slot + 4u * c);
      const int nin = (int)min(hdr.x, CAP);
      pend = chunk_hits(v, 2 - 4 * (int)c, nin + 2 - 4 * (int)c, q, P.th, hds);
      e_al = (uint64_t)hdr.y - 2ull;
    }
    WAVE_SYNC();
    emit_hits<SL, TAP>(ix, out, sw, g.read, g.base0, tg, e_al, c, pend, hds);
  }
}

__device__ __forceinline__ void pipe_begin_read(ScanWave& sw)
{
  sw.it_next = min((sw.it_next + 15u) & ~15u, sw.it_end);
  sw.rd_start = sw.it_next;
  sw.n_st = 0;
  sw.cur_seg = 0;
  sw.filt0 = 0xFFFFFFFFu, sw.filt1 = 0xFFFFFFFFu;
}
__device__ __forceinline__ void pipe_end_read(const BatchOut& out, ScanWave& sw, lds_u32* meta)
{
  flush_stage(out, sw);
  uint32_t f0 = sw.filt0, f1 = sw.filt1;
#pragma unroll
  for (int d = 32; d >= 1; d >>= 1) {
    f0 = min(f0, (uint32_t)__shfl_xor(f0, d));
    f1 = min(f1, (uint32_t)__shfl_xor(f1, d));
  }
  if (lane_id() == 0) {
    meta[0 * kReadChunk] = sw.rd_start;
    meta[1 * kReadChunk] = sw.it_next - sw.rd_start;
    meta[3 * kReadChunk] = f0;
    meta[4 * kReadChunk] = f1;
  }
}

template <int LOG_G, int CPL, int DEPTH, int WPE, bool SL, bool TAP>
__global__ __launch_bounds__(kScanWaves* kWave, WPE) void kr_scan_pipe_kernel_t(DevIndex ix, DevParams P, BatchIn in, BatchOut out)
{
  constexpr uint32_t PPS = 64u >> LOG_G;
  static_assert((kListCap / PPS) * CPL <= 64, "one hit bit per (pass, chunk)");
  __shared__ uint32_t s_row[kScanWaves][2][kListCap], s_q[kScanWaves][2][kListCap], s_tag[kScanWaves][2][kListCap], s_queue[kScanWaves][64];
  __shared__ uint32_t s_meta[kScanWaves][5 * kReadChunk];
  __shared__ __attribute__((aligned(16))) uint64_t s_stage[kScanWaves][kItemStage];
  __shared__ __attribute__((aligned(16))) uint4 s_fetab[KR_SCAN_PIPE_FE == 2 ? 1024 : 1];
  static_assert(kReadChunk <= 64, "one lane per read of a visit");
  if (KR_SCAN_PIPE_FE == 2) {
    fe_tab_to_lds(ix, (lds_u32x4*)s_fetab);
    __syncthreads();
  }
  const uint32_t w = threadIdx.x / kWave;
  SlotList LA{(lds_u32*)s_row[w][0], (lds_u32*)s_q[w][0], (lds_u32*)s_tag[w][0]};
  SlotList LB{(lds_u32*)s_row[w][1], (lds_u32*)s_q[w][1], (lds_u32*)s_tag[w][1]};
  lds_u32* queue = (lds_u32*)s_queue[w];
  lds_u32* meta = (lds_u32*)s_meta[w];
  ScanWave sw;
  sw.it_next = sw.it_end = sw.rd_start = 0;
  sw.err = 0;
  sw.cur_seg = 0;
  sw.n_st = 0;
  sw.stage = (lds_u64*)s_stage[w];
  sw.filt0 = sw.filt1 = 0xFFFFFFFFu;
  ReadCursor rc;
  rc.init(out.cursors + kCurScan * kCursors * kCursorStride, in.nreads, blockIdx.x * kScanWaves + w);
  uint32_t r0v, r1v;
  GroupGen<SL, KR_SCAN_PIPE_FE> gen;
  gen.tab = (const lds_u32x4*)s_fetab;
  uint4 v[DEPTH * CPL];
  while (rc.next(r0v, r1v)) {
    const uint32_t r0 = (uint32_t)__builtin_amdgcn_readfirstlane((int)r0v), r1 = (uint32_t)__builtin_amdgcn_readfirstlane((int)r1v);
    gen.init(r0, r1);
    GroupDesc ga, gb;
    bool flip = false;
    bool has_a = gen.next(ix, P, in, LA, meta, ga);
    if (has_a) {
      gen.prefetch(ix, in);
      pipe_begin_read(sw);
      pipe_issue<LOG_G, CPL, DEPTH, SL>(ix, LA, ga.nact, 0, v);
    }
    uint32_t c = 0;
    uint64_t hitbits = 0;
    bool has_b = false;
    while (has_a) {
      const SlotList& A = flip ? LB : LA;
      const SlotList& B = flip ? LA : LB;
      if (c == 0) {
        has_b = gen.next(ix, P, in, B, meta, gb);
        if (has_b) gen.prefetch(ix, in);
      }
      hitbits |= pipe_test<LOG_G, CPL, DEPTH, SL, TAP>(ix, P, out, sw, A, ga, c, v);
      const uint32_t npass = (ga.nact + PPS - 1u) / PPS;
// ... 27 lines not shown
```

### krepp_amd/csrc/kr_host_index.inc

```

struct kr_index {
  int device = 0;
  uint32_t log_g = 0;
  uint32_t slot_log2w = 0;
  DevIndex dix;
  std::vector<DevLib> hlibs;
  std::vector<void*> allocs;
  std::vector<kr_index_buffer> bufs;
  std::vector<uint8_t> desc;
  uint64_t bytes = 0;
  mutable std::mutex chain_mu;
  static constexpr uint32_t kChainEvents = 16;
  mutable hipEvent_t chain_ev[kChainEvents] = {nullptr};
  mutable uint32_t chain_n = 0;
  mutable bool chain_off = false;
  mutable std::mutex llh_mu;
  mutable DevBuf<double> llh_dev;
  mutable PinBuf<double> llh_pin;
  mutable DevBuf<char> d_names;
  mutable DevBuf<uint32_t> d_name_off;
};

namespace {

struct DescHeader {
  uint32_t magic, k, h, m, nlibs, tree_nnodes, nleaves, log_g;
  uint32_t slot_log2w, occ;
  uint64_t res_mask;
  uint8_t ppos[32], npos[32];
};
struct DescLib {
  uint64_t nkmers, nlist;
  uint32_t nrows, nsubsets, nnodes, numer;
};

int dev_alloc(kr_index* ix, void** p, uint64_t bytes)
{
  HIP_TRY(hipMalloc(p, bytes ? bytes : 16));
  ix->allocs.push_back(*p);
  ix->bytes += bytes;
  return KR_OK;
}

int alloc_from_desc(kr_index* ix, const DescHeader& H, const std::vector<DescLib>& L)
{
  ix->hlibs.resize(H.nlibs);
  ix->bufs.clear();
  for (uint32_t i = 0; i < H.nlibs; ++i) {
    DevLib& d = ix->hlibs[i];
    memset(&d, 0, sizeof(d));
    d.nkmers = L[i].nkmers, d.nlist = L[i].nlist, d.nrows = L[i].nrows, d.nsubsets = L[i].nsubsets, d.nnodes = L[i].nnodes,
    d.numer = L[i].numer;
    void* p;
    int rc;
    uint64_t b;
    b = (uint64_t)d.nrows * 8;
    if ((rc = dev_alloc(ix, &p, b))) return rc;
    d.bkt = (const uint64_t*)p;
    ix->bufs.push_back({p, b});
    b = (d.nkmers + 16) * 4;
    if ((rc = dev_alloc(ix, &p, b))) return rc;
    d.enc = (const uint32_t*)p;
    ix->bufs.push_back({p, b});
    b = (d.nkmers + 16) * 4;
    if ((rc = dev_alloc(ix, &p, b))) return rc;
    d.se = (const uint32_t*)p;
    ix->bufs.push_back({p, b});
    b = (uint64_t)d.nsubsets * 8;
    if ((rc = dev_alloc(ix, &p, b))) return rc;
    d.pse = (const uint2*)p;
    ix->bufs.push_back({p, b});
    b = (uint64_t)d.nnodes * 8;
    if ((rc = dev_alloc(ix, &p, b))) return rc;
    d.rho = (const double*)p;
    ix->bufs.push_back({p, b});
    b = d.nlist * 4;
    if ((rc = dev_alloc(ix, &p, b))) return rc;
    d.leaflist = (const uint32_t*)p;
    ix->bufs.push_back({p, b});
    if (H.occ) {
      b = (((uint64_t)d.nrows + 31) / 32) * 4;
      if ((rc = dev_alloc(ix, &p, b))) return rc;
      d.occ = (const uint32_t*)p;
      ix->bufs.push_back({p, b});
    }
    d.slot_log2w = H.slot_log2w;
    if (H.slot_log2w) {
      b = (uint64_t)d.nrows * slot_words(H.slot_log2w) * 4;
      if ((rc = dev_alloc(ix, &p, b))) return rc;
      d.slots = (const uint32_t*)p;
      ix->bufs.push_back({p, b});
    }
    if (H.slot_log2w == kSlotFilter) {
      b = (uint64_t)d.nrows * kFiltSlotCodes * 8;
      if ((rc = dev_alloc(ix, &p, b))) return rc;
      d.sx = (const uint2*)p;
      ix->bufs.push_back({p, b});
    }
  }
  void* p;
  int rc;
  uint64_t b = ((uint64_t)H.tree_nnodes + 1) * 4;
  if ((rc = dev_alloc(ix, &p, b))) return rc;
  ix->dix.node_info = (const uint32_t*)p;
  ix->bufs.push_back({p, b});
  b = (uint64_t)std::max<uint32_t>(1u, H.nleaves) * 4;
  if ((rc = dev_alloc(ix, &p, b))) return rc;
  ix->dix.leaf_se = (const uint32_t*)p;
  ix->bufs.push_back({p, b});
  ix->dix.nleaves = H.nleaves;
  ix->log_g = H.log_g;
  ix->slot_log2w = H.slot_log2w;
  b = (uint64_t)H.m * 4;
  if ((rc = dev_alloc(ix, &p, b))) return rc;
  ix->dix.res_lib = (const int32_t*)p;
  ix->bufs.push_back({p, b});
  b = (uint64_t)H.nlibs * sizeof(DevLib);
  if ((rc = dev_alloc(ix, &p, b))) return rc;
  ix->dix.libs = (const DevLib*)p;
  HIP_TRY(hipMemcpy(p, ix->hlibs.data(), b, hipMemcpyHostToDevice));
  ix->dix.lib0 = ix->hlibs[0];
  ix->dix.res_mask = H.res_mask;

  ix->dix.k = H.k, ix->dix.h = H.h, ix->dix.m = H.m, ix->dix.nlibs = H.nlibs, ix->dix.tree_nnodes = H.tree_nnodes;
  ix->dix.m_shift = 0xFFFFFFFFu;
  if ((H.m & (H.m - 1)) == 0) {
    uint32_t s = 0;
    while ((1u << s) < H.m) ++s;
    ix->dix.m_shift = s;
  }
  std::vector<uint8_t> pasc(H.ppos, H.ppos + H.h), nasc(H.npos, H.npos + (H.k - H.h));
  ix->dix.pmask = make_pext(pasc);
  ix->dix.nmask = make_pext(nasc);
  std::sort(pasc.begin(), pasc.end());
  std::sort(nasc.begin(), nasc.end());
  auto pack_desc = [](const std::vector<uint8_t>& asc, uint64_t (&out)[2]) {
    out[0] = out[1] = 0;
    for (size_t i = 0; i < asc.size(); ++i) out[i / 12] |= (uint64_t)asc[asc.size() - 1 - i] << (5 * (i % 12));
  };
  pack_desc(pasc, ix->dix.ppk);
  pack_desc(nasc, ix->dix.npk);
  {
    std::vector<uint4> tab(4 * 256, make_uint4(0, 0, 0, 0));
    std::vector<int> p_of(32, -1), n_of(32, -1);
    for (size_t t = 0; t < pasc.size(); ++t) p_of[pasc[t]] = (int)t;
    for (size_t t = 0; t < nasc.size(); ++t) n_of[nasc[t]] = (int)t;
    for (uint32_t b = 0; b < 4; ++b)
// ... 62 lines not shown
        if (a == 0 || a >= n) return Info{1, 0, 0};
        return a < se ? inf[a] : Info{0, 0, 0};
      };
      const Info A = part(pse[se].x), B = part(pse[se].y);
      Info r{0, 0, 0};
      if (A.kind && B.kind) {
        if (A.cnt == 0) r = B;
        else if (B.cnt == 0) r = A;
        else if (A.kind == 1 && B.kind == 1 && (uint64_t)A.lo + A.cnt == B.lo) r = Info{1, A.lo, A.cnt + B.cnt};
        else if (A.kind == 1 && B.kind == 1 && (uint64_t)B.lo + B.cnt == A.lo) r = Info{1, B.lo, A.cnt + B.cnt};
        else if ((uint64_t)A.cnt + B.cnt <= flat_max && lists.size() + flat_max < (1ull << 31)) {
          ranks_of(A, ta), ranks_of(B, tb2);
          const uint32_t off = (uint32_t)lists.size();
          std::set_union(ta.begin(), ta.end(), tb2.begin(), tb2.end(), std::back_inserter(lists));
          r = Info{2, off, (uint32_t)lists.size() - off};
        }
      }
      if (r.kind == 1 && r.cnt >= 2 && r.cnt < run_min) r.kind = 0;
      if (r.kind && !flat_max) r.kind = 0;
      inf[se] = r;
      cls[se] = se | ((r.kind ? 3u : 2u) << 30);
    }
  }
  for (uint32_t se = 0; se < n; ++se) {
    if ((cls[se] >> 30) == 3u) {
      pse[se] = make_uint2(inf[se].lo | (inf[se].kind == 2 ? 0x80000000u : 0u), inf[se].cnt);
    } else {
      const uint32_t a = pse[se].x, b = pse[se].y;
      pse[se] = make_uint2(a < n ? cls[a] : 0u, b < n ? cls[b] : 0u);
    }
  }
}

int kr_debug_colour_classes(const uint32_t* pse_pairs, uint32_t nsubsets, const uint8_t* node_kind, uint32_t tree_nnodes,
                            uint32_t* cls_out, uint32_t* pse_out, uint32_t* lists_out, uint64_t* nlist)
{
  kr::clear_error();
  if (!pse_pairs || !node_kind || !cls_out || !pse_out || !nlist) return kr::fail(KR_ERR_ARG, "kr_debug_colour_classes: null argument");
  std::vector<uint32_t> node_info(tree_nnodes + 1, 0);
  uint32_t rank = 0;
  for (uint32_t se = 1; se <= tree_nnodes; ++se) {
    const uint32_t kd = node_kind[se] & 3u;
    node_info[se] = kd;
    if (kd == 1) node_info[se] |= rank++ << 2;
  }
  std::vector<uint2> pse(nsubsets);
  for (uint32_t i = 0; i < nsubsets; ++i) pse[i] = make_uint2(pse_pairs[2 * i], pse_pairs[2 * i + 1]);
  std::vector<uint32_t> cls, lists;
  colour_classes(pse, node_info, tree_nnodes, cls, lists);
  for (uint32_t i = 0; i < nsubsets; ++i) cls_out[i] = cls[i], pse_out[2 * i] = pse[i].x, pse_out[2 * i + 1] = pse[i].y;
  const uint64_t cap = *nlist;
  *nlist = lists.size();
  if (lists.size() > cap || (!lists_out && !lists.empty())) return kr::fail(KR_ERR_CAPACITY, "kr_debug_colour_classes: list buffer too small");
  if (!lists.empty()) memcpy(lists_out, lists.data(), lists.size() * 4);
  return KR_OK;
}

int kr_index_upload(const kr_index_view* v, int device, uint32_t flags, kr_index** out)
{
  kr::clear_error();
  if (!v || !out || !v->libs || !v->ppos || !v->npos || !v->node_kind) return kr::fail(KR_ERR_ARG, "kr_index_upload: null argument");
  *out = nullptr;
  if (v->k < 3 || v->k > 31 || v->h == 0 || v->h >= v->k || v->k - v->h > 16 || v->h > 15)
    return kr::fail(KR_ERR_ARG, "kr_index_upload: unsupported k/h (need k<=31, k-h<=16, h<=15)");
  if (v->nlibs == 0 || v->nlibs > (uint32_t)kMaxLibs) return kr::fail(KR_ERR_ARG, "kr_index_upload: 1..16 partial libraries supported");
  if (v->m == 0 || v->m > 65536) return kr::fail(KR_ERR_ARG, "kr_index_upload: m out of range");
  if (v->tree_nnodes >= (1u << 30)) return kr::fail(KR_ERR_ARG, "kr_index_upload: tree too large");
  int ndev = 0;
  if (hipGetDeviceCount(&ndev) != hipSuccess || ndev <= 0) return kr::fail(KR_ERR_NO_DEVICE, "no HIP device available");
  if (device < 0 || device >= ndev) return kr::fail(KR_ERR_ARG, "kr_index_upload: bad device ordinal");
  HIP_TRY(hipSetDevice(device));

  DescHeader H;
  memset(&H, 0, sizeof(H));
  H.magic = kDescMagic, H.k = v->k, H.h = v->h, H.m = v->m, H.nlibs = v->nlibs, H.tree_nnodes = v->tree_nnodes;
  memcpy(H.ppos, v->ppos, v->h);
  memcpy(H.npos, v->npos, v->k - v->h);
  std::vector<DescLib> L(v->nlibs);
  std::vector<int32_t> res_lib(v->m, -1);
  for (uint32_t i = 0; i < v->nlibs; ++i) {
    const kr_lib_view& lv = v->libs[i];
    if (lv.r >= v->m) return kr::fail(KR_ERR_FORMAT, "library residue r >= m");
    if (lv.nnodes != v->tree_nnodes + 1) return kr::fail(KR_ERR_FORMAT, "crecord nnodes does not match the tree");
    L[i] = DescLib{lv.nkmers, 0, lv.nrows, lv.nsubsets, lv.nnodes, lv.frac ? lv.r + 1 : 1u};
    if (lv.frac)
      for (uint32_t q = 0; q <= lv.r; ++q) res_lib[q] = (int32_t)i;
    else
      res_lib[lv.r] = (int32_t)i;
  }
  for (uint32_t q = 0; q < v->m && q < 64; ++q)
    if (res_lib[q] >= 0) H.res_mask |= 1ull << q;
  std::vector<uint32_t> node_info(v->tree_nnodes + 1, 0), leaf_se;
  for (uint32_t se = 1; se <= v->tree_nnodes; ++se) {
    uint32_t kd = v->node_kind[se] & 3u;
    node_info[se] = kd;
    if (kd == 1) {
      node_info[se] |= (uint32_t)leaf_se.size() << 2;
      leaf_se.push_back(se);
    }
  }
  H.nleaves = (uint32_t)leaf_se.size();
  if (2ull * H.nleaves > 131072) return kr::fail(KR_ERR_ARG, "kr_index_upload: more than 65536 reference leaves is not supported");
  {
    double nk = 0, nr = 0;
    for (uint32_t i = 0; i < v->nlibs; ++i) nk += (double)v->libs[i].nkmers, nr += (double)v->libs[i].nrows;
    double mean_len = nr > 0 ? nk / nr : 0;
    H.log_g = mean_len <= 3.0 ? 0u : (mean_len <= 44.0 ? 2u : 3u);
    if (const char* e = getenv("KR_LOG_G")) H.log_g = (uint32_t)atoi(e) > 3 ? 3u : (uint32_t)atoi(e);
    if (H.log_g == 1) H.log_g = 2;
    bool fits32 = true;
    for (uint32_t i = 0; i < v->nlibs; ++i) fits32 = fits32 && v->libs[i].nkmers < (1ull << 32);
    const double need = mean_len + 3.0 * std::sqrt(mean_len);
    if (mean_len >= 12.0 && fits32) H.slot_log2w = need <= 30.0 ? 5u : (need <= 62.0 ? 6u : (need <= 126.0 ? 7u : 0u));
    const bool want_filter = getenv("KR_SLOT_FILTER") ? atoi(getenv("KR_SLOT_FILTER")) != 0 : kFilterByDefault;
    if (H.slot_log2w == 6u && want_filter) H.slot_log2w = kSlotFilter;
    H.occ = (mean_len < 1.0 && !H.slot_log2w) ? 1u : 0u;
    if (const char* e = getenv("KR_OCC_BITMAP")) H.occ = atoi(e) ? 1u : 0u;
    if (const char* e = getenv("KR_SLOT_LOG2W")) {
      const uint32_t w = (uint32_t)atoi(e);
      H.slot_log2w = (fits32 && w >= 5 && w <= 9) ? w : 0u;
    }
  }
  std::vector<std::vector<uint2>> hpse(v->nlibs);
  std::vector<std::vector<uint32_t>> cls(v->nlibs), lists(v->nlibs);
  for (uint32_t i = 0; i < v->nlibs; ++i) {
    const kr_lib_view& lv = v->libs[i];
    if (lv.nsubsets > kColMask) return kr::fail(KR_ERR_ARG, "kr_index_upload: more than 2^30 colours is not supported");
    hpse[i].resize(lv.nsubsets);
    if (lv.nsubsets) {
      if (flags & KR_VIEW_DEVICE)
        HIP_TRY(hipMemcpy(hpse[i].data(), lv.pse, (uint64_t)lv.nsubsets * 8, hipMemcpyDeviceToHost));
      else
        memcpy(hpse[i].data(), lv.pse, (uint64_t)lv.nsubsets * 8);
    }
    colour_classes(hpse[i], node_info, v->tree_nnodes, cls[i], lists[i]);
    L[i].nlist = lists[i].size();
  }
  std::unique_ptr<kr_index> ix(new kr_index());
  ix->device = device;
  ix->chain_off = getenv("KR_NO_KERNEL_CHAIN") != nullptr;
  int rc = alloc_from_desc(ix.get(), H, L);
  if (rc) {
    kr_index_free(ix.release());
    return rc;
  }
  const hipMemcpyKind kind = (flags & KR_VIEW_DEVICE) ? hipMemcpyDeviceToDevice : hipMemcpyHostToDevice;
  HIP_TRY(hipMemcpy((void*)ix->dix.node_info, node_info.data(), node_info.size() * 4, hipMemcpyHostToDevice));
  if (!leaf_se.empty()) HIP_TRY(hipMemcpy((void*)ix->dix.leaf_se, leaf_se.data(), leaf_se.size() * 4, hipMemcpyHostToDevice));
  DevBuf<uint32_t> b_bad;
  if (!b_bad.reserve(1)) return alloc_failed("kr_index_upload");
  uint32_t* d_bad = b_bad.get();
  HIP_TRY(hipMemset(d_bad, 0, 4));
  for (uint32_t i = 0; i < v->nlibs; ++i) {
    const kr_lib_view& lv = v->libs[i];
    const DevLib& d = ix->hlibs[i];
    const uint32_t* src_cmer = lv.cmer;
    const uint64_t* src_inc = lv.inc;
    DevBuf<uint64_t> t_cmer, t_inc;
    if (!(flags & KR_VIEW_DEVICE)) {
      if (!t_cmer.reserve(lv.nkmers + 2)) return alloc_failed("kr_index_upload: staging");
      HIP_TRY(hipMemcpy(t_cmer.get(), lv.cmer, lv.nkmers * 8, hipMemcpyHostToDevice));
      if (!t_inc.reserve((uint64_t)lv.nrows + 2)) return alloc_failed("kr_index_upload: staging");
      HIP_TRY(hipMemcpy(t_inc.get(), lv.inc, (uint64_t)lv.nrows * 8, hipMemcpyHostToDevice));
      src_cmer = (const uint32_t*)t_cmer.get();
      src_inc = t_inc.get();
    }
    HIP_TRY(hipMemset((void*)d.enc, 0xFF, (d.nkmers + 16) * 4));
    HIP_TRY(hipMemset((void*)d.se, 0, (d.nkmers + 16) * 4));
    if (lv.nsubsets > kColMask) return kr::fail(KR_ERR_ARG, "kr_index_upload: more than 2^30 colours is not supported");
    DevBuf<uint32_t> b_cls;
    if (!b_cls.reserve((uint64_t)lv.nsubsets + 4)) return alloc_failed("kr_index_upload: staging");
    uint32_t* d_cls = b_cls.get();
    if (lv.nsubsets) HIP_TRY(hipMemcpy(d_cls, cls[i].data(), (uint64_t)lv.nsubsets * 4, hipMemcpyHostToDevice));
    if (!lists[i].empty()) HIP_TRY(hipMemcpy((void*)d.leaflist, lists[i].data(), lists[i].size() * 4, hipMemcpyHostToDevice));
    if (lv.nkmers)
      hipLaunchKernelGGL(kr_relayout_cmer, dim3(2048), dim3(256), 0, 0, src_cmer, lv.nkmers, (uint32_t*)d.enc, (uint32_t*)d.se, d_cls, lv.nsubsets);
    if (lv.nrows) hipLaunchKernelGGL(kr_relayout_inc, dim3(1024), dim3(256), 0, 0, src_inc, lv.nrows, (uint64_t*)d.bkt, d_bad);
    if (lv.nrows && H.occ) hipLaunchKernelGGL(kr_build_occ, dim3(1024), dim3(256), 0, 0, d.bkt, lv.nrows, (uint32_t*)d.occ);
    if (lv.nrows && H.slot_log2w == kSlotFilter) {
      hipLaunchKernelGGL(kr_build_fslots, dim3(8192), dim3(256), 0, 0, d.bkt, d.enc, lv.nrows, (uint4*)d.slots);
      hipLaunchKernelGGL(kr_build_sx, dim3(8192), dim3(256), 0, 0, d.bkt, d.enc, d.se, lv.nrows, (uint2*)d.sx);
    } else if (lv.nrows && H.slot_log2w)
      hipLaunchKernelGGL(kr_build_slots, dim3(8192), dim3(256), 0, 0, d.bkt, d.enc, lv.nrows, slot_words(H.slot_log2w), (uint32_t*)d.slots);
    HIP_TRY(hipDeviceSynchronize());
    t_cmer.reset(), t_inc.reset(), b_cls.reset();
    if (lv.nsubsets) HIP_TRY(hipMemcpy((void*)d.pse, hpse[i].data(), (uint64_t)lv.nsubsets * 8, hipMemcpyHostToDevice));
    HIP_TRY(hipMemcpy((void*)d.rho, lv.rho, (uint64_t)lv.nnodes * 8, kind));
  }
  uint32_t bad = 0;
  HIP_TRY(hipMemcpy(&bad, d_bad, 4, hipMemcpyDeviceToHost));
  if (bad) {
    kr_index_free(ix.release());
    return kr::fail(KR_ERR_FORMAT, "inc-* is not monotone or a bucket exceeds 2^24 entries / 2^40 offset");
  }
  HIP_TRY(hipMemcpy((void*)ix->dix.res_lib, res_lib.data(), (uint64_t)v->m * 4, hipMemcpyHostToDevice));
  *out = ix.release();
  return KR_OK;
}

void kr_index_free(kr_index* ix)
{
  if (!ix) return;
  (void)hipSetDevice(ix->device);
  for (void* p : ix->allocs) (void)hipFree(p);
  for (auto& e : ix->chain_ev)
    if (e) (void)hipEventDestroy(e);
  delete ix;
}

uint64_t kr_index_device_bytes(const kr_index* ix) { return ix ? ix->bytes : 0; }
uint32_t kr_index_slot_words(const kr_index* ix) { return ix && ix->slot_log2w ? slot_words(ix->slot_log2w) : 0; }
uint32_t kr_index_slot_format(const kr_index* ix) { return ix ? ix->slot_log2w : 0; }

int kr_index_export(const kr_index* ix, void* desc, uint64_t* desc_bytes, kr_index_buffer* bufs, uint32_t* nbufs)
{
  if (!ix || !desc_bytes || !nbufs) return kr::fail(KR_ERR_ARG, "kr_index_export: null argument");
  uint64_t need = ix->desc.size();
  uint32_t nb = (uint32_t)ix->bufs.size();
  bool fits = desc && *desc_bytes >= need && bufs && *nbufs >= nb;
  *desc_bytes = need;
  *nbufs = nb;
  if (!fits) return (desc || bufs) ? kr::fail(KR_ERR_ARG, "kr_index_export: buffers too small") : KR_OK;
  memcpy(desc, ix->desc.data(), need);
  memcpy(bufs, ix->bufs.data(), nb * sizeof(kr_index_buffer));
  return KR_OK;
}

int kr_index_import(const void* desc, uint64_t desc_bytes, int device, kr_index** out, kr_index_buffer* bufs, uint32_t* nbufs)
{
  kr::clear_error();
  if (!desc || !out || !nbufs || desc_bytes < sizeof(DescHeader)) return kr::fail(KR_ERR_ARG, "kr_index_import: bad argument");
  DescHeader H;
  memcpy(&H, desc, sizeof(H));
  if (H.magic != kDescMagic || desc_bytes != sizeof(H) + (uint64_t)H.nlibs * sizeof(DescLib) || H.nlibs == 0 || H.nlibs > (uint32_t)kMaxLibs)
    return kr::fail(KR_ERR_FORMAT, "kr_index_import: bad descriptor");
  std::vector<DescLib> L(H.nlibs);
  memcpy(L.data(), (const uint8_t*)desc + sizeof(H), H.nlibs * sizeof(DescLib));
  int ndev = 0;
  if (hipGetDeviceCount(&ndev) != hipSuccess || ndev <= 0) return kr::fail(KR_ERR_NO_DEVICE, "no HIP device available");
  if (device < 0 || device >= ndev) return kr::fail(KR_ERR_ARG, "kr_index_import: bad device ordinal");
  HIP_TRY(hipSetDevice(device));
  std::unique_ptr<kr_index> ix(new kr_index());
  ix->device = device;
  ix->chain_off = getenv("KR_NO_KERNEL_CHAIN") != nullptr;
  int rc = alloc_from_desc(ix.get(), H, L);
  if (rc) {
    kr_index_free(ix.release());
    return rc;
  }
  uint32_t nb = (uint32_t)ix->bufs.size();
  if (!bufs || *nbufs < nb) {
    *nbufs = nb;
    kr_index_free(ix.release());
    return kr::fail(KR_ERR_ARG, "kr_index_import: bufs too small");
  }
  memcpy(bufs, ix->bufs.data(), nb * sizeof(kr_index_buffer));
  *nbufs = nb;
  *out = ix.release();
  return KR_OK;
}

}

namespace {

struct Rccl {
  void* h = nullptr;
  decltype(&ncclCommInitAll) CommInitAll = nullptr;
  decltype(&ncclCommDestroy) CommDestroy = nullptr;
  decltype(&ncclBroadcast) Broadcast = nullptr;
  decltype(&ncclGroupStart) GroupStart = nullptr;
  decltype(&ncclGroupEnd) GroupEnd = nullptr;
  decltype(&ncclGetErrorString) GetErrorString = nullptr;
  std::string err;
  bool load()
  {
    if (h) return true;
    const char* names[] = {getenv("KR_RCCL_LIB"), "librccl.so.1", "librccl.so", "/opt/rocm/lib/librccl.so.1"};
    for (const char* n : names)
      if (n && *n && (h = dlopen(n, RTLD_NOW | RTLD_GLOBAL))) break;
    if (!h) {
      err = std::string("cannot load RCCL: ") + (dlerror() ? dlerror() : "librccl.so.1 not found");
      return false;
    }
#define KR_SYM(field, name)                                                            \
  if (!(field = reinterpret_cast<decltype(field)>(dlsym(h, name)))) {                  \
    err = std::string("RCCL lacks ") + name;                                           \
    dlclose(h), h = nullptr;                                                           \
    return false;                                                                      \
  }
    KR_SYM(CommInitAll, "ncclCommInitAll")
    KR_SYM(CommDestroy, "ncclCommDestroy")
    KR_SYM(Broadcast, "ncclBroadcast")
    KR_SYM(GroupStart, "ncclGroupStart")
    KR_SYM(GroupEnd, "ncclGroupEnd")
// ... 82 lines not shown
```

### krepp_amd/csrc/kr_host_stream.inc

```

constexpr uint32_t kMaxLanes = 8;
enum LaneEvent {
  kEvCopyIn = 0,
  kEvFirstKernel,
  kEvScanDone,
  kEvAccDone,
  kEvLastKernel,
  kEvAccStart,
  kEvLlhStart,
  kEvCount
};
struct Lane {
  hipStream_t stream = nullptr;
  hipEvent_t ev[kEvCount] = {};
  BatchIn in;
  BatchOut out;
  uint32_t* d_counters = nullptr;
  uint32_t* d_cursors = nullptr;
  ulonglong2* d_dd = nullptr;
  uint32_t dd_slots = 0;
  uint32_t* d_dd_direct = nullptr;
  double2* d_dd_dv = nullptr;
  uint32_t* d_dd_ohist = nullptr;
  uint8_t* d_dd_oslot = nullptr;
// ... 281 lines not shown
      !reserve_all(c, t.d_vtile, t.d_rfirst, t.d_real_off, t.d_real_cnt, t.d_real_onmers, t.d_real_na, t.d_real_roff, t.d_real_rcnt, t.d_choice, t.d_lread, t.d_vsrc) ||
      !reserve_all(2 * c, t.d_longs, t.d_tile_filt, t.d_real_filt) || !reserve_all(4 * blk_cap, t.d_bsum) || !reserve_all(4, t.d_sum, t.h_sum))
    return alloc_failed("build_tiles_device");
  hipStream_t st = s->lanes[0].stream;
  TileLayIO io;
  io.bases = bases, io.offsets = offsets;
  io.nreads = nreads, io.k = s->ix->dix.k, io.tile_min_pos = s->tile_min_pos;
  io.spare = s->max_reads - nreads;
  io.nblk = nblk;
  io.bsum_e = t.d_bsum.get(), io.bsum_v = io.bsum_e + blk_cap, io.bsum_b = io.bsum_v + blk_cap, io.bsum_l = io.bsum_b + blk_cap;
  io.choice = t.d_choice.get(), io.lread = t.d_lread.get(), io.vsrc = t.d_vsrc.get();
  io.voff = t.d_voff.get(), io.vtile = t.d_vtile.get(), io.rfirst = t.d_rfirst.get(), io.longs = t.d_longs.get();
  io.sum = t.d_sum.get();
  io.dst = nullptr;
  const dim3 bgrid(std::min<uint32_t>(nblk, 4096u));
  hipLaunchKernelGGL(kr_tile_lay_count_kernel, bgrid, dim3(256), 0, st, io);
  hipLaunchKernelGGL(kr_tile_lay_escan_kernel, dim3(1), dim3(1024), 0, st, io);
  hipLaunchKernelGGL(kr_tile_lay_choose_kernel, bgrid, dim3(256), 0, st, io);
  hipLaunchKernelGGL(kr_tile_lay_lscan_kernel, dim3(1), dim3(1024), 0, st, io);
  hipLaunchKernelGGL(kr_tile_lay_reads_kernel, bgrid, dim3(256), 0, st, io);
  hipLaunchKernelGGL(kr_tile_lay_tiles_kernel, dim3(std::min<uint32_t>((nreads + 3) / 4, 8192u)), dim3(256), 0, st, io);
  HIP_TRY(hipGetLastError());
  HIP_TRY(hipMemcpyAsync(t.h_sum.get(), t.d_sum.get(), 3 * sizeof(uint64_t), hipMemcpyDeviceToHost, st));
  HIP_TRY(hipStreamSynchronize(st));
  const uint64_t nv = t.h_sum.get()[0], nlong = t.h_sum.get()[1], nb = t.h_sum.get()[2];
  if (nlong == 0) return KR_OK;
  if (nv > s->max_reads) return kr::fail(KR_ERR_ARG, "kr_batch_submit: the device offsets do not ascend");
  if (nb + 256 > t.d_bases.size() && !t.d_bases.reserve(nb + nb / 4 + 256)) {
    t.h_bases.reset();
    return alloc_failed("build_tiles_device");
  }
  io.dst = t.d_bases.get();
  hipLaunchKernelGGL(kr_tile_lay_copy_kernel, dim3((uint32_t)std::min<uint64_t>((nv + 3) / 4, 16384u)), dim3(256), 0, st, io);
  HIP_TRY(hipGetLastError());
  t.nv = (uint32_t)nv, t.nlong = (uint32_t)nlong, t.on_device = true;
  *tiled = true;
  return KR_OK;
}

template <typename F>
void with_bools(F&& f)
{
  f();
}
template <typename F, typename... Bs>
void with_bools(F&& f, bool b, Bs... rest)
{
  auto bind = [&](auto c) { with_bools([&](auto... cs) { f(c, cs...); }, rest...); };
  b ? bind(std::true_type{}) : bind(std::false_type{});
}
template <int V>
using int_c = std::integral_constant<int, V>;
template <typename F>
void with_scan_shape(uint32_t slot_log2w, uint32_t log_g, F&& f)
{
  switch (slot_log2w) {
    case 5: return f(int_c<2>{}, int_c<2>{}, std::true_type{});
    case 6: return f(int_c<2>{}, int_c<4>{}, std::true_type{});
    case 7: return f(int_c<3>{}, int_c<4>{}, std::true_type{});
    case 8: return f(int_c<2>{}, int_c<3>{}, std::true_type{});
  }
  switch (log_g) {
    case 0: return f(int_c<0>{}, int_c<2>{}, std::false_type{});
    case 2: return f(int_c<2>{}, int_c<3>{}, std::false_type{});
    default: return f(int_c<3>{}, int_c<3>{}, std::false_type{});
  }
}

TileBatch tile_batch(const kr_stream* s)
{
  const kr_stream::Tiles& tl = s->tiles;
  return TileBatch{tl.d_vtile.get(), tl.d_longs.get(), tl.d_rfirst.get(), tl.d_tile_filt.get(), tl.nv, tl.nlong, s->nreads,
                   tl.d_real_off.get(), tl.d_real_cnt.get(), tl.d_real_onmers.get(), tl.d_real_filt.get(), tl.d_real_na.get(),
                   s->rows_mode ? tl.d_real_roff.get() : nullptr, s->rows_mode ? tl.d_real_rcnt.get() : nullptr};
}

void launch_scan(kr_stream* s, Lane& L, bool single, bool tap)
{
  hipStream_t st = L.stream;
  const DevIndex& dix = s->ix->dix;
  BatchOut& o = L.out;
  const dim3 block(kScanWaves * kWave);
  auto grid = [&](uint32_t blocks) { return dim3(std::min<uint32_t>((L.nreads + kScanWaves - 1) / kScanWaves, blocks)); };
  static const bool pipe = !getenv("KR_SCAN_PIPE") || atoi(getenv("KR_SCAN_PIPE")) != 0;
  with_bools([&](auto SL, auto TAP) {
    if (s->fk) {
      hipLaunchKernelGGL((kr_scan_filt_kernel_t<KR_SCAN_FILT_DEPTH, KR_SCAN_FILT_WPE, SL.value, TAP.value>), grid(s->scan_filt_blocks), block, 0, st, dix, s->dp, L.in, o);
      return;
    }
    with_scan_shape(s->ix->slot_log2w, s->ix->log_g, [&](auto LG, auto CP, auto SLOTTED) {
      if constexpr (SLOTTED.value)
        if (pipe) {
          hipLaunchKernelGGL((kr_scan_pipe_kernel_t<LG.value, CP.value, KR_SCAN_DEPTH, KR_SCAN_PIPE_WPE, SL.value, TAP.value>), grid(s->scan_pipe_blocks), block, 0, st, dix, s->dp, L.in, o);
          return;
        }
      hipLaunchKernelGGL((kr_scan_kernel_t<LG.value, CP.value, SL.value, TAP.value, SLOTTED.value>), grid(s->scan_blocks), block, 0, st, dix, s->dp, L.in, o);
    });
  }, single, tap);
}

void launch_accumulate(kr_stream* s, Lane& L, bool single)
{
  hipStream_t st = L.stream;
  const DevIndex& dix = s->ix->dix;
  BatchOut& o = L.out;
  const uint32_t nreads = L.nreads;
  const kr_stream::Tiles& tl = s->tiles;
  const TileBatch tb = tile_batch(s);
  if (tl.active)
    hipLaunchKernelGGL(kr_tile_filt_kernel, dim3(std::min<uint32_t>((tl.nv + 255) / 256, 4096u)), dim3(256), 0, st, o, tb);
  const uint32_t lds = probe_lds_bytes(s->dp.np, o.bm_words), lds_lean = probe_lds_bytes(s->dp.np, o.bm_words, true);
  const uint32_t lds_lean2 = probe_lds_bytes(s->dp.np, o.bm_words, true, 2);
  static const bool no_lean2 = getenv("KR_DEBUG_NO_LEAN2") != nullptr;
  const uint32_t grid_lean2 = (lds_lean2 <= 65536u && !no_lean2) ? std::min(nreads, s->nwaves_lean2) : 0u;
  const uint32_t grid_lean = std::min(nreads, s->nwaves_lean), grid_full = std::min(nreads, s->nwaves_full);
  const bool np5 = s->dp.np == 5 && !getenv("KR_DEBUG_NP0");
  with_bools([&](auto SL, auto NP5, auto FK) {
    constexpr int NPV = NP5.value ? 5 : 0;
    hipLaunchKernelGGL((kr_acc_kernel_t<SL.value, NPV, false, 7, FK.value>), dim3(grid_lean), dim3(kWave), lds_lean, st, dix, s->dp, L.in, o);
    if (grid_lean2)
      hipLaunchKernelGGL((kr_acc_kernel_t<SL.value, NPV, false, 8, FK.value>), dim3(grid_lean2), dim3(kWave), lds_lean2, st, dix, s->dp, L.in, o);
    hipLaunchKernelGGL((kr_acc_kernel_t<SL.value, NPV, true, 7, FK.value>), dim3(grid_full), dim3(kWave), lds, st, dix, s->dp, L.in, o);
  }, single, np5, s->fk);
  if (tl.active) {
    const uint32_t W = std::min<uint32_t>(32u, s->nwaves / std::max<uint32_t>(1u, tl.nlong));
    if (W >= 2 && tl.nlong <= s->nwaves) {
      hipLaunchKernelGGL(kr_tile_add_kernel, dim3(tl.nlong * W), dim3(kWave), 0, st, dix, s->dp, o, tb, W);
      hipLaunchKernelGGL(kr_tile_merge_kernel<true>, dim3(tl.nlong), dim3(kWave), (o.bm_words * 4u + 15u) & ~15u, st, dix, s->dp, o, tb);
    } else {
      hipLaunchKernelGGL(kr_tile_merge_kernel<false>, dim3(std::min<uint32_t>(tl.nlong, s->nwaves)), dim3(kWave), (o.bm_words * 4u + 15u) & ~15u, st,
                         dix, s->dp, o, tb);
    }
  }
}

void launch_likelihood(kr_stream* s, Lane& L)
{
  hipStream_t st = L.stream;
  const DevIndex& dix = s->ix->dix;
  BatchOut& o = L.out;
  const bool np5 = s->llh.th == 4, direct = np5 && o.dd_nodes;
  const uint32_t places = kDdOslots * kDdClasses * o.dd_nodes;
  hipLaunchKernelGGL(kr_dedup_clear_kernel, dim3(4096), dim3(256), 0, st, o);
  if (o.dd_nodes) hipLaunchKernelGGL(kr_dedup_oslot_kernel, dim3(std::min<uint32_t>((L.nreads + 4095) / 4096, 1024u)), dim3(256), 0, st, o, L.nreads);
  hipLaunchKernelGGL(kr_dedup_kernel, dim3(kDedupBlocks), dim3(256), 0, st, o);
  if (direct) hipLaunchKernelGGL(kr_dedup_direct_kernel, dim3(std::min<uint32_t>((places + 4095u) / 4096u, 4096u)), dim3(256), 0, st, o);
  with_bools([&](auto NP5) {
    constexpr int NPV = NP5.value ? 5 : 0;
    hipLaunchKernelGGL(kr_llh_pre_kernel<NPV>, dim3(4096), dim3(256), 0, st, s->llh, dix, o);
    hipLaunchKernelGGL(kr_llh_kernel<NPV>, dim3(2048), dim3(256), 0, st, s->llh, dix, o);
  }, np5);
  if (direct) hipLaunchKernelGGL(kr_dedup_dv_kernel, dim3(std::min<uint32_t>((places + 1023u) / 1024u, 4096u)), dim3(256), 0, st, o);
}

void launch_select(kr_stream* s, Lane& L)
{
  hipStream_t st = L.stream;
  const DevIndex& dix = s->ix->dix;
  BatchOut& o = L.out;
  const uint32_t nreads = L.nreads;
  const uint32_t sgrid = std::min<uint32_t>((nreads + 7) / 8, 16384u);
  const bool filt = !s->dp.no_filter && s->dp.multi;
  static const bool lane_sel = !getenv("KR_SELECT_LANE") || atoi(getenv("KR_SELECT_LANE")) != 0;
  const uint32_t lgrid = std::min<uint32_t>((nreads + 255) / 256, 8192u);
  with_bools([&](auto NP5, auto FILT) {
    constexpr int NPV = NP5.value ? 5 : 0;
    if (!FILT.value && lane_sel)
// ... 464 lines not shown
        HIP_TRY(hipMemcpyAsync(t.d_voff.get(), t.h_voff.get(), ((uint64_t)t.nv + 1) * 8, hipMemcpyHostToDevice, st));
        HIP_TRY(hipMemcpyAsync(t.d_vtile.get(), t.h_vtile.get(), t.nv, hipMemcpyHostToDevice, st));
        HIP_TRY(hipMemcpyAsync(t.d_rfirst.get(), t.h_rfirst.get(), (uint64_t)nreads * 4, hipMemcpyHostToDevice, st));
        HIP_TRY(hipMemcpyAsync(t.d_longs.get(), t.h_longs.get(), (uint64_t)t.nlong * 8, hipMemcpyHostToDevice, st));
      }
      L.in.bases = t.d_bases.get();
      L.in.offsets = t.d_voff.get();
      L.nreads = t.nv;
    } else if (flags & KR_BASES_DEVICE) {
      L.in.bases = bases;
      L.in.offsets = offsets + r0;
    } else {
      const uint64_t b0 = offsets[r0] - offsets[0], b1 = offsets[r1] - offsets[0];
      const uint64_t* ho = s->h_offsets;
      const uint8_t* src = bases + offsets[r0];
      if (!(flags & KR_BASES_PINNED)) {
        memcpy(s->h_bases + b0, src, b1 - b0);
        src = s->h_bases + b0;
      }
      if ((flags & KR_BASES_PINNED) && offsets[0] == 0)
        ho = offsets;
      else
        for (uint32_t r = r0; r <= r1; ++r) s->h_offsets[r] = offsets[r] - offsets[0];
      HIP_TRY(hipMemcpyAsync(s->d_bases + b0, src, b1 - b0, hipMemcpyHostToDevice, st));
      HIP_TRY(hipMemcpyAsync(s->d_offsets + r0 + l, ho + r0, ((uint64_t)(r1 - r0) + 1) * 8, hipMemcpyHostToDevice, st));
      L.in.bases = s->d_bases;
      L.in.offsets = s->d_offsets + r0 + l;
    }
    if (s->text.req && (!s->tiles.active || s->rows_mode) && !s->text.ids_on_device) {
      HIP_TRY(hipMemcpyAsync(s->text.d_ids, s->text.h_ids, s->text.id_bytes, hipMemcpyHostToDevice, st));
      HIP_TRY(hipMemcpyAsync(s->text.d_id_off, s->text.h_id_off, ((uint64_t)nreads + 1) * 4, hipMemcpyHostToDevice, st));
    }
    L.in.nreads = L.nreads;
    BatchOut& o = L.out;
    o = s->out;
    o.counters = L.d_counters, o.cursors = L.d_cursors;
    o.dd_table = L.d_dd, o.dd_slots = L.dd_slots;
    o.dd_direct = L.d_dd_direct, o.dd_dv = L.d_dd_dv, o.dd_ohist = L.d_dd_ohist, o.dd_oslot = L.d_dd_oslot;
    o.g_planes = L.d_g_planes, o.g_counts = L.d_g_counts, o.g_list = L.d_g_list, o.stk_spill = L.d_stk;
    o.rd_off += r0, o.rd_cnt += r0, o.rd_onmers += r0, o.rd_filt += 2ull * r0, o.rd_na += r0;
    o.rd_it_off += r0, o.rd_it_cnt += r0;
    o.long_list += r0 + 16ull * s->nwaves * l;
    o.items += (uint64_t)l * lane_item_cap, o.item_cap = lane_item_cap;
    const uint64_t rb = L.rec_base;
    o.rec_read += rb, o.rec_key += rb, o.rec_hist += rb, o.rec_d += rb, o.rec_v += rb, o.rec_chisq += rb, o.rec_sel += rb;
    o.rec_w0 += rb, o.rec_rep += rb, o.rep_list += rb + (uint64_t)l * kRepSlack, o.rep_dv += rb + (uint64_t)l * kRepSlack;
    o.rec_cap = lane_rec_cap;
    o.rep_cap = (uint32_t)std::min<uint64_t>((uint64_t)lane_rec_cap + kRepSlack, 0xFFFFFFFFull);
    o.keep_v = ((flags & KR_ROWS_ONLY) && !(flags & KR_TAP_ACCS)) ? 0u : 1u;
    o.hist_always = (flags & KR_TAP_ACCS) ? 1u : 0u;
    o.v_tile = s->tiles.active ? s->tiles.d_vtile.get() : nullptr;
    o.rows_mode = s->rows_mode ? 1u : 0u;
    o.rd_rcnt += r0, o.rd_roff += r0, o.row_bsum += r0 / kRowBlock + 2ull * l;
    o.row_key = o.rec_rep, o.row_d = reinterpret_cast<double*>(o.rep_dv);
    o.rows_indexed = s->rows_indexed ? 1u : 0u;
    if (s->rows_indexed)
      o.row_key = reinterpret_cast<uint32_t*>(o.rec_d), o.row_dix = o.row_key + lane_rec_cap, o.dist_list = o.rec_v;
    return launch_lane(s, L, flags);
  };
  for (uint32_t l = 0; l < P; ++l) {
    const int rc = submit_lane(l);
    if (rc) {
      const std::string msg = kr_last_error();
      for (uint32_t j = 0; j <= l; ++j)
        if (s->lanes[j].stream) (void)hipStreamSynchronize(s->lanes[j].stream);
      (void)hipGetLastError();
      s->nlanes = 0;
      s->nrecs = 0, s->nhits = 0;
      s->waited = true;
      s->batch_rc = rc;
      s->batch_msg = msg;
      return kr::fail(rc, msg);
    }
  }
  return KR_OK;
}

enum CounterCombine { kSum, kMax, kOr };
struct CounterRule {
  CounterSlot slot;
  CounterCombine how;
};
constexpr CounterRule kCounterRules[] = {
  {kCtErr, kOr}, {kCtL2Reads, kSum}, {kCtTapHits, kSum}, {kCtRecords, kSum},
  {kCtStEvents, kSum}, {kCtStKeys, kSum}, {kCtStBatches, kSum}, {kCtStBig, kSum}, {kCtStLevelTiles, kSum}, {kCtStMaxKeys, kMax}, {kCtStMaxEvents, kMax},
  {kCtCycLevel, kSum}, {kCtCycFinalize, kSum}, {kCtCycRead, kSum},
  {kCtProblems, kSum}, {kCtStackSpills, kSum}, {kCtTileHoles, kSum},
};

constexpr int kItemPlacementTrials = 5;
int item_placement_step(kr_stream* s)
{
  kr_stream::ItemPlacement& ip = s->ipl;
  if (ip.trials_left < 0) {
    const char* e = getenv("KR_ITEM_PLACEMENT_TRIALS");
    ip.trials_left = (e && *e) ? std::max(0, atoi(e)) : kItemPlacementTrials;
  }
  if (ip.trials_left == 0 && !ip.aside.get()) return KR_OK;
  if (s->tiles.active || s->nreads < 1000000u || (s->flags & KR_TAP_HITS)) return KR_OK;
  float ms = 0;
  for (uint32_t l = 0; l < s->nlanes; ++l) {
    float ml = 0;
    if (hipEventElapsedTime(&ml, s->lanes[l].ev[kEvFirstKernel], s->lanes[l].ev[kEvScanDone]) != hipSuccess) {
      (void)hipGetLastError();
      return KR_OK;
    }
    ms += ml;
  }
  const double ns = (double)ms * 1e6 / s->nreads;
  static const bool verbose = getenv("KR_ITEM_PLACEMENT_VERBOSE") != nullptr;
  if (ip.settling > 0) {
    --ip.settling;
    if (verbose) fprintf(stderr, "[krepp_amd] item list: early launch %.3f ns per read (not measured)\n", ns);
    return KR_OK;
  }
  if (ip.aside.get()) {
    const bool better = ns < ip.best_ns * 0.985;
    if (verbose) fprintf(stderr, "[krepp_amd] item list trial %u: %.3f ns per read against %.3f: %s\n", ip.tried, ns, ip.best_ns, better ? "kept" : "dropped");
    if (better) {
      ip.best_ns = ns, ++ip.kept_new;
    } else {
      s->items.swap(ip.aside);
      s->out.items = s->items.get();
    }
    ip.aside.reset();
  } else {
    ip.best_ns = ns;
    if (verbose) fprintf(stderr, "[krepp_amd] item list as allocated: %.3f ns per read\n", ns);
  }
  if (ip.trials_left > 0) {
    --ip.trials_left;
    const uint64_t bytes = (uint64_t)s->item_cap * sizeof(uint2);
    size_t free_b = 0, total_b = 0;
    if (hipMemGetInfo(&free_b, &total_b) != hipSuccess || free_b < 2 * bytes) {
      (void)hipGetLastError();
      ip.trials_left = 0;
      return KR_OK;
    }
    if (!ip.aside.renew(s->item_cap)) {
      (void)hipGetLastError();
      ip.trials_left = 0;
      return KR_OK;
    }
    s->items.swap(ip.aside);
    s->out.items = s->items.get();
    ip.settling = 1;
    ++ip.tried;
  }
  return KR_OK;
}

int kr_batch_wait(kr_stream* s)
{
  if (!s || !s->submitted) return kr::fail(KR_ERR_STATE, "kr_batch_wait: nothing submitted");
  if (s->waited) return s->batch_rc ? kr::fail(s->batch_rc, s->batch_msg) : KR_OK;
  HIP_TRY(hipSetDevice(s->ix->device));
  memset(s->h_counters, 0, sizeof(s->h_counters));
  uint32_t extent = 0;
  bool lane_full = false;
  for (uint32_t l = 0; l < s->nlanes; ++l) {
    Lane& L = s->lanes[l];
    HIP_TRY(hipStreamSynchronize(L.stream));
    const uint32_t* c = L.h_counters;
    L.nrecs = std::min(c[kCtRecSlots], L.rec_cap);
    L.nrows = c[kCtRows];
    extent = std::max(extent, L.nrecs ? L.rec_base + L.nrecs : 0u);
    lane_full = lane_full || c[kCtRecSlots] > L.rec_cap;
// ... 185 lines not shown
      HIP_TRY(hipMemcpyAsync(s->h_rec_d.get() + hoff, o.rec_d, nc * 8, hipMemcpyDeviceToHost, st));
      if (full) {
        HIP_TRY(hipMemcpyAsync(s->h_rec_v.get() + hoff, o.rec_v, nc * 8, hipMemcpyDeviceToHost, st));
        s->d2h_bytes += nc * 8;
        if (!s->dp.no_filter && s->dp.multi) {
          HIP_TRY(hipMemcpyAsync(s->h_rec_chisq.get() + hoff, o.rec_chisq, nc * 8, hipMemcpyDeviceToHost, st));
          s->d2h_bytes += nc * 8;
        } else
          std::fill(s->h_rec_chisq.get() + hoff, s->h_rec_chisq.get() + hoff + nc, std::numeric_limits<double>::quiet_NaN());
        if (s->flags & KR_TAP_ACCS)
          for (uint32_t x = 0; x < s->dp.np; ++x) {
            HIP_TRY(hipMemcpyAsync(s->h_rec_hist.get() + (uint64_t)x * hist_stride_host + hoff, o.rec_hist + (uint64_t)x * s->rec_cap, nc * 4, hipMemcpyDeviceToHost, st));
            s->d2h_bytes += nc * 4;
          }
      }
    }
    copies_started = true;
    hoff += nc;
  }
  if ((s->flags & KR_TAP_HITS) && s->waited && s->nhits)
    HIP_TRY(hipMemcpyAsync(s->h_hits.get(), s->out.hits, s->nhits * sizeof(kr_hit), hipMemcpyDeviceToHost, s->lanes[0].stream));
  int rc = kr_batch_wait(s);
  for (uint32_t l = 0; l < s->nlanes; ++l) HIP_TRY(hipStreamSynchronize(s->lanes[l].stream));
  if (rc) return rc;
  lap("copies to the host");
  for (uint32_t l = 0; l < s->nlanes; ++l) {
    const Lane& L = s->lanes[l];
    const uint32_t delta = rows_mode ? (uint32_t)L.host_off : (uint32_t)L.host_off - L.rec_base;
    if (!delta) continue;
    uint32_t* off = s->h_rd_off + L.read0;
    const uint32_t* cnt = s->h_rd_cnt + L.read0;
    for (uint32_t r = 0; r < L.nreads; ++r) off[r] = cnt[r] ? off[r] + delta : 0u;
  }
  s->collected = true;
  fill_view(s, v, false);
  v->nrecs = (uint32_t)hoff;
  v->rec_hist_stride = hoff;
  if (rows_mode) {
    if (s->h_sel_ones < hoff) {
      const uint64_t a0 = s->h_sel_ones, len = hoff - a0;
      const int nt = (int)std::max<uint64_t>(1, std::min<uint64_t>((uint64_t)std::min(kr::parallel_width(), 16), len >> 22));
      kr::parallel_for(nt, [&](int t) {
        const uint64_t a = a0 + len * (uint64_t)t / nt, b = a0 + len * (uint64_t)(t + 1) / nt;
        memset(s->h_rec_sel.get() + a, 1, b - a);
      });
      s->h_sel_ones = hoff;
    }
    v->nrows = hoff;
  } else {
    const int nt = (int)std::max<uint64_t>(1, std::min<uint64_t>((uint64_t)std::min(kr::parallel_width(), 16), hoff >> 20));
    std::vector<uint64_t> part((size_t)nt, 0);
    const uint8_t* sel = s->h_rec_sel.get();
    kr::parallel_for(nt, [&](int t) {
      uint64_t a = hoff * (uint64_t)t / nt, b = hoff * (uint64_t)(t + 1) / nt, c = 0;
      for (uint64_t i = a; i < b; ++i) c += sel[i];
      part[(size_t)t] = c;
    });
    uint64_t nrows = 0;
    for (uint64_t c : part) nrows += c;
    v->nrows = nrows;
  }
  lap("offsets + row count");
  return KR_OK;
}

int kr_batch_collect_device(kr_stream* s, kr_result_view* v)
{
  kr::clear_error();
  if (!s || !v) return kr::fail(KR_ERR_ARG, "kr_batch_collect_device: null argument");
  int rc = kr_batch_wait(s);
  if (rc) return rc;
  fill_view(s, v, true);
  return KR_OK;
}

int kr_batch_hits(kr_stream* s, const kr_hit** hits, uint64_t* nhits)
{
  if (!s || !hits || !nhits || !s->waited) return kr::fail(KR_ERR_STATE, "kr_batch_hits: collect a KR_TAP_HITS batch first");
  *hits = s->h_hits.get();
  *nhits = s->nhits;
  return KR_OK;
}

int kr_batch_readtaps(kr_stream* s, const kr_readtap** taps)
{
  if (!s || !taps || !s->waited) return kr::fail(KR_ERR_STATE, "kr_batch_readtaps: collect a batch first");
  *taps = reinterpret_cast<const kr_readtap*>(s->h_rd_filt);
  return KR_OK;
}

int kr_debug_stream_move(kr_stream* s, int which)
{
  if (!s || (s->submitted && !s->waited)) return kr::fail(KR_ERR_STATE, "kr_debug_stream_move: wait for the batch first");
  HIP_TRY(hipSetDevice(s->device));
  BatchOut& o = s->out;
  Lane& L = s->lanes[0];
  const uint64_t mr = s->max_reads, ML = s->max_lanes;
  int rc = 0;
#define MV(ptr, n)   if ((rc = salloc(s, &ptr, (n)))) return rc;
  switch (which) {
    case 0: MV(o.items, s->item_cap); break;
    case 1:
      MV(o.rd_off, mr); MV(o.rd_cnt, mr); MV(o.rd_onmers, mr); MV(o.rd_filt, 2 * mr); MV(o.rd_na, mr);
      MV(o.rd_it_off, mr); MV(o.rd_it_cnt, mr); MV(o.long_list, mr + 16ull * s->nwaves * ML);
      break;
    case 2: MV(L.d_counters, kCounterWords); MV(L.d_cursors, kCurSets * kCursors * kCursorStride); break;
    case 3:
      MV(o.rec_read, s->rec_cap); MV(o.rec_key, s->rec_cap); MV(o.rec_d, s->rec_cap); MV(o.rec_sel, s->rec_cap);
      MV(o.rec_w0, s->rec_cap); MV(o.rec_rep, s->rec_cap); MV(o.rep_list, (uint64_t)s->rec_cap + (uint64_t)kMaxLanes * kRepSlack); MV(o.rep_dv, (uint64_t)s->rec_cap + (uint64_t)kMaxLanes * kRepSlack);
      MV(L.d_dd, L.dd_slots);
      break;
    case 4: {
      hipStream_t st = nullptr;
      HIP_TRY(hipStreamCreateWithFlags(&st, hipStreamNonBlocking));
      s->moved_streams.push_back(L.stream);
      L.stream = st;
      break;
    }
    default: return kr::fail(KR_ERR_ARG, "kr_debug_stream_move: which = 0 .. 4");
  }
#undef MV
  return KR_OK;
}

int kr_debug_stream_addrs(kr_stream* s, uint64_t* out8)
{
  if (!s || !out8) return kr::fail(KR_ERR_ARG, "kr_debug_stream_addrs: null argument");
  const BatchOut& o = s->out;
  const Lane& L = s->lanes[0];
  const void* p[8] = {o.items, L.d_counters, L.d_cursors, o.rd_off, o.rd_it_off, o.rd_filt, o.rec_key, L.d_dd};
  for (int i = 0; i < 8; ++i) out8[i] = (uint64_t)(uintptr_t)p[i];
  return KR_OK;
}

int kr_debug_item_placement(kr_stream* s, uint32_t* tried, uint32_t* kept, double* best_ns_per_read)
{
  if (!s) return kr::fail(KR_ERR_ARG, "kr_debug_item_placement: null argument");
  if (tried) *tried = s->ipl.tried;
  if (kept) *kept = s->ipl.kept_new;
  if (best_ns_per_read) *best_ns_per_read = s->ipl.best_ns;
  return KR_OK;
}

int kr_batch_timing(kr_stream* s, kr_timing* t)
{
  if (!s || !t || !s->waited) return kr::fail(KR_ERR_STATE, "kr_batch_timing: wait for a batch first");
  memset(t, 0, sizeof(*t));
  float first = 0, last = 0;
  for (uint32_t l = 0; l < s->nlanes; ++l) {
    Lane& L = s->lanes[l];
    float a = 0;
    HIP_TRY(hipEventElapsedTime(&a, L.ev[kEvCopyIn], L.ev[kEvFirstKernel]));
    t->ms_h2d += a;
    HIP_TRY(hipEventElapsedTime(&a, L.ev[kEvFirstKernel], L.ev[kEvScanDone]));
    t->ms_scan += a;
    HIP_TRY(hipEventElapsedTime(&a, L.ev[kEvAccStart], L.ev[kEvAccDone]));
    t->ms_acc += a;
    HIP_TRY(hipEventElapsedTime(&a, L.ev[kEvLlhStart], L.ev[kEvLastKernel]));
    t->ms_llh += a;
    if (l) {
      HIP_TRY(hipEventElapsedTime(&a, s->lanes[0].ev[kEvFirstKernel], L.ev[kEvFirstKernel]));
      first = std::min(first, a);
    }
    HIP_TRY(hipEventElapsedTime(&a, s->lanes[0].ev[kEvFirstKernel], L.ev[kEvLastKernel]));
    last = std::max(last, a);
  }
// ... 50 lines not shown
```

Measured before the change: 125.0 million reads/s.

## Embed dictionary-coded colour ids in slot tail to skip se lookups

At index upload, a histogram of colour keys is built and the most frequent (up to 65535) get 16-bit codes. These codes are packed into the unused tail words of each slot row, and a dictionary of codes is appended after the se array. During scan, each hit loads the matching code pair from the same slot row and, when a code exists, points the item index at the small dictionary instead of the per-kmer se entry. This aims to replace scattered HBM reads of se with cache-friendly dictionary reads, at the cost of an extra 8-byte load per probe and more index-build work.

```diff
diff --git a/include/krepp_amd.h b/include/krepp_amd.h
--- a/include/krepp_amd.h
+++ b/include/krepp_amd.h
@@ -78,6 +78,7 @@
 KR_API uint64_t kr_index_device_bytes(const kr_index*);
 KR_API uint32_t kr_index_slot_words(const kr_index*);
 KR_API uint32_t kr_index_slot_format(const kr_index*);
+KR_API int kr_index_slot_colour_stats(const kr_index*, uint64_t* dict_codes, uint64_t* coded_entries, uint64_t* total_entries);
 
 KR_API int kr_index_broadcast(const kr_index* root, int ndev, const int* devices, kr_index** replicas);
 
@@ -147,6 +148,9 @@
   uint32_t se;
 } kr_hit;
 KR_API int kr_batch_hits(kr_stream*, const kr_hit** hits, uint64_t* nhits);
+KR_API int kr_debug_tap_coded_items(kr_stream*, uint64_t* coded);
+KR_API int kr_debug_slot_colour_layout(uint32_t n, uint32_t words, const uint32_t* counts, uint32_t nkeys, uint32_t limit, uint32_t* ncol,
+                                       uint32_t* order, uint32_t* norder);
 typedef struct kr_readtap {
   uint32_t hdist_filt[2];
 } kr_readtap;
diff --git a/krepp_amd/capi.py b/krepp_amd/capi.py
--- a/krepp_amd/capi.py
+++ b/krepp_amd/capi.py
@@ -89,11 +89,11 @@
 EXPORTS = [
     "kr_host_index_load", "kr_host_sketch_load", "kr_format_seek", "kr_build_sketch", "kr_host_index_free", "kr_host_index_view", "kr_host_index_node_name",
     "kr_host_index_node_label", "kr_host_index_node_parent", "kr_host_index_node_blen",
-    "kr_index_upload", "kr_index_free", "kr_index_export", "kr_index_import", "kr_index_device_bytes", "kr_index_slot_words", "kr_index_slot_format", "kr_index_broadcast",
+    "kr_index_upload", "kr_index_free", "kr_index_export", "kr_index_import", "kr_index_device_bytes", "kr_index_slot_words", "kr_index_slot_format", "kr_index_slot_colour_stats", "kr_index_broadcast",
     "kr_params_default", "kr_stream_create", "kr_stream_destroy", "kr_batch_submit", "kr_batch_wait",
     "kr_batch_collect", "kr_batch_collect_device", "kr_stream_text_enable", "kr_batch_submit_text", "kr_batch_collect_text",
     "kr_stream_fastq_enable", "kr_batch_submit_fastq", "kr_batch_fastq_names", "kr_debug_fastq_batch", "kr_debug_tile_layout", "kr_debug_tile_shape", "kr_batch_hits", "kr_batch_readtaps",
-    "kr_debug_front_end", "kr_debug_stream_move", "kr_debug_stream_addrs", "kr_debug_item_placement", "kr_debug_brent", "kr_debug_prefix", "kr_debug_colour_classes", "kr_llh_batch", "kr_llh_eval_indexed", "kr_batch_timing",
+    "kr_debug_front_end", "kr_debug_stream_move", "kr_debug_stream_addrs", "kr_debug_item_placement", "kr_debug_brent", "kr_debug_prefix", "kr_debug_colour_classes", "kr_debug_tap_coded_items", "kr_debug_slot_colour_layout", "kr_llh_batch", "kr_llh_eval_indexed", "kr_batch_timing",
     "kr_place_tree_create", "kr_place_tree_create_lineage", "kr_place_tree_nnodes", "kr_place_summary_add",
     "kr_place_summary_text", "kr_place_tree_free", "kr_place_tree_kinds", "kr_place_batch", "kr_place_stream", "kr_place_frame", "kr_place_counters",
     "kr_debug_last_d2h_bytes", "kr_debug_place_fixed5", "kr_place_text_counters", "kr_place_path_counters", "kr_fastx_open", "kr_fastx_open_at", "kr_fastx_next", "kr_fastx_detach", "kr_fastx_release", "kr_fastx_close", "kr_fastx_parallel_chunks", "kr_fastx_pgz_stats", "kr_format_dist", "kr_debug_fixed5", "kr_free", "kr_host_alloc", "kr_host_free",
@@ -143,6 +143,9 @@
     lib.kr_index_slot_words.argtypes = [vp]
     lib.kr_index_slot_format.argtypes = [vp]
     lib.kr_index_slot_format.restype = C.c_uint32
+    lib.kr_index_slot_colour_stats.argtypes = [vp, u64p, u64p, u64p]
+    lib.kr_debug_tap_coded_items.argtypes = [vp, u64p]
+    lib.kr_debug_slot_colour_layout.argtypes = [C.c_uint32, C.c_uint32, vp, C.c_uint32, C.c_uint32, u32p, vp, u32p]
     lib.kr_debug_stream_move.argtypes = [vp, C.c_int]
     lib.kr_debug_stream_addrs.argtypes = [vp, u64p]
     lib.kr_debug_item_placement.argtypes = [vp, u32p, u32p, C.POINTER(C.c_double)]
@@ -340,6 +343,12 @@
     def slot_format(self):
         return int(self.lib.kr_index_slot_format(self.h))
 
+    @property
+    def slot_colour_stats(self):
+        d, c, t = C.c_uint64(), C.c_uint64(), C.c_uint64()
+        check(self.lib.kr_index_slot_colour_stats(self.h, C.byref(d), C.byref(c), C.byref(t)))
+        return int(d.value), int(c.value), int(t.value)
+
     def stream(self, params=None, max_reads=1 << 16, max_bases=None, max_records=0):
         return Stream(self, params or default_params(), max_reads, max_bases or max_reads * 160, max_records)
 
@@ -479,6 +488,11 @@
         raw = C.string_at(p, n.value * C.sizeof(KrHit))
         return np.frombuffer(raw, dtype=dt).copy()
 
+    def tap_coded_items(self):
+        n = C.c_uint64()
+        check(self.lib.kr_debug_tap_coded_items(self.h, C.byref(n)))
+        return int(n.value)
+
     def readtaps(self, nreads):
         p = u32p()
         check(self.lib.kr_batch_readtaps(self.h, C.byref(p)))
@@ -634,6 +648,20 @@
     total = C.c_uint64(0)
     check(load().kr_debug_prefix(values.ctypes.data, len(values), block, width, prefix.ctypes.data, C.byref(total)))
     return prefix, total.value
+
+
+def slot_ncol(n, words):
+    out = C.c_uint32()
+    check(load().kr_debug_slot_colour_layout(int(n), int(words), None, 0, 0, C.byref(out), None, None))
+    return int(out.value)
+
+
+def slot_colour_ranking(counts, limit=65535):
+    counts = np.ascontiguousarray(counts, dtype=np.uint32)
+    order = np.zeros(max(1, len(counts)), np.uint32)
+    n = C.c_uint32()
+    check(load().kr_debug_slot_colour_layout(0, 64, counts.ctypes.data, len(counts), int(limit), None, order.ctypes.data, C.byref(n)))
+    return order[:n.value].copy()
 
 
 def colour_classes(pse, node_kind):
diff --git a/krepp_amd/csrc/kr_common.h b/krepp_amd/csrc/kr_common.h
--- a/krepp_amd/csrc/kr_common.h
+++ b/krepp_amd/csrc/kr_common.h
@@ -3,6 +3,7 @@
 
 #include "krepp_amd.h"
 
+#include <algorithm>
 #include <atomic>
 #include <cmath>
 #include <cstdio>
@@ -120,6 +121,30 @@
   return (size_t)snprintf(out, 64, "%.5f", v);
 }
 
+constexpr uint32_t kSlotColourDict = 65536u;
+constexpr uint32_t kSlotNoCode = 0xFFFFu;
+KR_HD inline uint32_t slot_ncol(uint32_t n, uint32_t W)
+{
+  const uint32_t room = 2u * W > 2u * n + 6u ? 2u * W - 2u * n - 6u : 0u;
+  return n < room ? n : room;
+}
+KR_HD inline uint32_t slot_colour_key(uint32_t tagged, uint32_t nleaves) { return (tagged >> 30) == 1u ? (tagged & 0x3FFFFFFFu) : nleaves + (tagged & 0x3FFFFFFFu); }
+inline std::vector<uint32_t> slot_colour_ranking(const uint32_t* counts, uint32_t nkeys, uint32_t limit)
+{
+  std::vector<uint32_t> order;
+  for (uint32_t i = 0; i < nkeys; ++i)
+    if (counts[i]) order.push_back(i);
+  limit = limit < kSlotNoCode ? limit : kSlotNoCode;
+  auto before = [&](uint32_t a, uint32_t b) { return counts[a] != counts[b] ? counts[a] > counts[b] : a < b; };
+  if (order.size() > limit) {
+    std::partial_sort(order.begin(), order.begin() + limit, order.end(), before);
+    order.resize(limit);
+  } else {
+    std::sort(order.begin(), order.end(), before);
+  }
+  return order;
+}
+
 inline uint64_t fmix64(uint64_t v)
 {
   v ^= v >> 33;
diff --git a/krepp_amd/csrc/kr_dev_common.inc b/krepp_amd/csrc/kr_dev_common.inc
--- a/krepp_amd/csrc/kr_dev_common.inc
+++ b/krepp_amd/csrc/kr_dev_common.inc
@@ -49,6 +49,7 @@
   uint64_t nkmers, nlist;
   uint32_t nrows, nsubsets, nnodes, numer;
   uint32_t slot_log2w;
+  uint32_t slot_colours;
 };
 
 struct DevIndex {
@@ -87,6 +88,7 @@
   kCtRecords = 4,
   kCtLlhCursor = 5,
   kCtItemSlots = 6,
+  kCtTapCoded = 7,
   kCtStEvents = 9,
   kCtStKeys = 10,
   kCtStBatches = 11,
diff --git a/krepp_amd/csrc/kr_dev_likelihood.inc b/krepp_amd/csrc/kr_dev_likelihood.inc
--- a/krepp_amd/csrc/kr_dev_likelihood.inc
+++ b/krepp_amd/csrc/kr_dev_likelihood.inc
@@ -1232,8 +1232,32 @@
   }
 }
 
-__global__ void kr_build_slots(const uint64_t* bkt, const uint32_t* enc, uint32_t nrows, uint32_t words, uint32_t* slots)
-{
+constexpr uint32_t kHistLds = 12288u;
+__global__ __launch_bounds__(1024) void kr_colour_hist(const uint32_t* se, uint64_t n, uint32_t nleaves, uint32_t nkeys, uint32_t* cnt, uint32_t* val)
+{
+  __shared__ uint32_t s_cnt[kHistLds];
+  for (uint32_t i = threadIdx.x; i < kHistLds; i += blockDim.x) s_cnt[i] = 0u;
+  __syncthreads();
+  for (uint64_t i = blockIdx.x * (uint64_t)blockDim.x + threadIdx.x; i < n; i += (uint64_t)gridDim.x * blockDim.x) {
+    const uint32_t t = se[i], key = kr::slot_colour_key(t, nleaves);
+    if (key >= nkeys) continue;
+    if (key < kHistLds) {
+      if (atomicAdd(&s_cnt[key], 1u) == 0u) val[key] = t;
+    } else if (atomicAdd(&cnt[key], 1u) == 0u) {
+      val[key] = t;
+    }
+  }
+  __syncthreads();
+  for (uint32_t i = threadIdx.x; i < kHistLds && i < nkeys; i += blockDim.x)
+    if (s_cnt[i]) atomicAdd(&cnt[i], s_cnt[i]);
+}
+
+__global__ void kr_build_slots(const uint64_t* bkt, const uint32_t* enc, uint32_t nrows, uint32_t words, uint32_t* slots, const uint32_t* se,
+                               const uint16_t* code_of, uint32_t nleaves, uint32_t nkeys, unsigned long long* ncoded)
+{
+  __shared__ uint32_t s_coded;
+  if (threadIdx.x == 0) s_coded = 0u;
+  __syncthreads();
   const uint64_t n = (uint64_t)nrows * words;
   for (uint64_t i = blockIdx.x * (uint64_t)blockDim.x + threadIdx.x; i < n; i += (uint64_t)gridDim.x * blockDim.x) {
     const uint32_t row = (uint32_t)(i / words), wd = (uint32_t)(i - (uint64_t)row * words);
@@ -1247,6 +1271,24 @@
       x = (uint32_t)st;
     else if (wd - 2u < ln)
       x = enc[st + wd - 2u];
+    else if (code_of) {
+      const uint32_t ncol = kr::slot_ncol(ln, words);
+      uint32_t got = 0;
+#pragma unroll
+      for (uint32_t half = 0; half < 2u; ++half) {
+        const uint32_t t = 2u * words - 1u - (2u * wd + half);
+        uint32_t code = kr::kSlotNoCode;
+        if (t >= 2u && t - 2u < ncol) {
+          const uint32_t key = kr::slot_colour_key(se[st + t - 2u], nleaves);
+          if (key < nkeys) code = code_of[key];
+        }
+        got += code != kr::kSlotNoCode ? 1u : 0u;
+        x = half ? (x & 0x0000FFFFu) | (code << 16) : (x & 0xFFFF0000u) | code;
+      }
+      if (got) atomicAdd(&s_coded, got);
+    }
     slots[i] = x;
   }
-}
+  __syncthreads();
+  if (threadIdx.x == 0 && s_coded && ncoded) atomicAdd(ncoded, (unsigned long long)s_coded);
+}
diff --git a/krepp_amd/csrc/kr_dev_scan.inc b/krepp_amd/csrc/kr_dev_scan.inc
--- a/krepp_amd/csrc/kr_dev_scan.inc
+++ b/krepp_amd/csrc/kr_dev_scan.inc
@@ -170,9 +170,17 @@
 }
 
 constexpr uint32_t kItemMarker = 0x80000000u;
+__device__ __forceinline__ uint2 slot_codes(uint2 pair, uint32_t c, uint32_t ncol)
+{
+  const int k = (int)ncol + 2 - 4 * (int)c;
+  if (k < 4) pair.x |= k < 3 ? 0xFFFFFFFFu : 0x0000FFFFu;
+  if (k < 2) pair.y |= k < 1 ? 0xFFFFFFFFu : 0x0000FFFFu;
+  return pair;
+}
 template <bool SL, bool TAP, bool FK = false>
 __device__ __forceinline__ void emit_hits(const DevIndex& ix, const BatchOut& out, ScanWave& sw, uint32_t read, uint32_t base0,
-                                          uint32_t tg, uint64_t e_al, uint32_t c, uint32_t pend, uint32_t hds)
+                                          uint32_t tg, uint64_t e_al, uint32_t c, uint32_t pend, uint32_t hds,
+                                          uint2 cpair = make_uint2(0xFFFFFFFFu, 0xFFFFFFFFu))
 {
   const uint64_t lt = (1ull << lane_id()) - 1ull;
   const uint32_t seg = base0 >> 7;
@@ -180,7 +188,9 @@
     const bool has = pend != 0;
     const uint32_t e = has ? (uint32_t)__ffs((int)pend) - 1u : 0u;
     const uint32_t hd = (hds >> (8u * e)) & 31u;
-    const uint64_t idx = e_al + 4ull * c + e;
+    uint64_t idx = e_al + 4ull * c + e;
+    const uint32_t code = (((e & 2u) ? cpair.x : cpair.y) >> ((e & 1u) ? 0u : 16u)) & 0xFFFFu;
+    const bool coded = !FK && has && code != kr::kSlotNoCode;
     if (has) {
       if (tag_strand(tg))
         sw.filt1 = min(sw.filt1, hd);
@@ -202,8 +212,10 @@
         } else {
           atomicOr(&out.counters[kCtErr], kErrHitCap);
         }
-      }
-    }
+        if (coded) atomicAdd(&out.counters[kCtTapCoded], 1u);
+      }
+    }
+    if (coded) idx = get_lib<SL>(ix, tag_lib(tg)).nkmers + 16ull + code;
     const uint64_t hm = __ballot(has);
     const uint32_t mark = seg != sw.cur_seg ? 1u : 0u;
     if (sw.n_st + (uint32_t)__popcll(hm) + mark > kItemStage) flush_stage(out, sw);
@@ -373,21 +385,25 @@
     WAVE_SYNC();
     uint32_t pend = 0, hds = 0, tg = 0, c = 0;
     uint64_t e_al = 0;
+    uint2 cpair = make_uint2(0xFFFFFFFFu, 0xFFFFFFFFu);
     if (lane < min(64u, H - w0)) {
       const uint32_t d = queue[lane], probe = d & 255u;
       c = d >> 8;
       const uint32_t row = (uint32_t)pl.bkt[probe];
       const uint32_t q = pl.q[probe];
       tg = pl.tag[probe];
-      const uint32_t* slot = get_lib<SL>(ix, tag_lib(tg)).slots + (uint64_t)row * W;
+      const DevLib Lb = get_lib<SL>(ix, tag_lib(tg));
+      const uint32_t* slot = Lb.slots + (uint64_t)row * W;
       const uint2 hdr = *reinterpret_cast<const uint2*>(slot);
       const uint4 v = *reinterpret_cast<const uint4*>(slot + 4u * c);
+      cpair = *reinterpret_cast<const uint2*>(slot + (W - 2u - 2u * c));
       const int nin = (int)min(hdr.x, CAP);
       pend = chunk_hits(v, 2 - 4 * (int)c, nin + 2 - 4 * (int)c, q, P.th, hds);
       e_al = (uint64_t)hdr.y - 2ull;
+      cpair = slot_codes(cpair, c, Lb.slot_colours ? kr::slot_ncol(hdr.x, W) : 0u);
     }
     WAVE_SYNC();
-    emit_hits<SL, TAP>(ix, out, sw, read, base0, tg, e_al, c, pend, hds);
+    emit_hits<SL, TAP>(ix, out, sw, read, base0, tg, e_al, c, pend, hds, cpair);
   }
 }
 
diff --git a/krepp_amd/csrc/kr_dev_scan_pipe.inc b/krepp_amd/csrc/kr_dev_scan_pipe.inc
--- a/krepp_amd/csrc/kr_dev_scan_pipe.inc
+++ b/krepp_amd/csrc/kr_dev_scan_pipe.inc
@@ -230,21 +230,25 @@
     WAVE_SYNC();
     uint32_t pend = 0, hds = 0, tg = 0, c = 0;
     uint64_t e_al = 0;
+    uint2 cpair = make_uint2(0xFFFFFFFFu, 0xFFFFFFFFu);
     if (lane < min(64u, H - w0)) {
       const uint32_t d = queue[lane], probe = d & 255u;
       c = d >> 8;
       const uint32_t row = L.row[probe];
       const uint32_t q = L.q[probe];
       tg = L.tag[probe];
-      const uint32_t* slot = get_lib<SL>(ix, tag_lib(tg)).slots + (uint64_t)row * W;
+      const DevLib Lb = get_lib<SL>(ix, tag_lib(tg));
+      const uint32_t* slot = Lb.slots + (uint64_t)row * W;
       const uint2 hdr = *reinterpret_cast<const uint2*>(slot);
       const uint4 v = *reinterpret_cast<const uint4*>(slot + 4u * c);
+      cpair = *reinterpret_cast<const uint2*>(slot + (W - 2u - 2u * c));
       const int nin = (int)min(hdr.x, CAP);
       pend = chunk_hits(v, 2 - 4 * (int)c, nin + 2 - 4 * (int)c, q, P.th, hds);
       e_al = (uint64_t)hdr.y - 2ull;
-    }
-    WAVE_SYNC();
-    emit_hits<SL, TAP>(ix, out, sw, g.read, g.base0, tg, e_al, c, pend, hds);
+      cpair = slot_codes(cpair, c, Lb.slot_colours ? kr::slot_ncol(hdr.x, W) : 0u);
+    }
+    WAVE_SYNC();
+    emit_hits<SL, TAP>(ix, out, sw, g.read, g.base0, tg, e_al, c, pend, hds, cpair);
   }
 }
 
diff --git a/krepp_amd/csrc/kr_host_index.inc b/krepp_amd/csrc/kr_host_index.inc
--- a/krepp_amd/csrc/kr_host_index.inc
+++ b/krepp_amd/csrc/kr_host_index.inc
@@ -26,12 +26,15 @@
 struct DescHeader {
   uint32_t magic, k, h, m, nlibs, tree_nnodes, nleaves, log_g;
   uint32_t slot_log2w, occ;
+  uint32_t slot_colours, reserved0;
   uint64_t res_mask;
   uint8_t ppos[32], npos[32];
 };
 struct DescLib {
   uint64_t nkmers, nlist;
   uint32_t nrows, nsubsets, nnodes, numer;
+  uint64_t ncoded;
+  uint32_t ndict, reserved0;
 };
 
 int dev_alloc(kr_index* ix, void** p, uint64_t bytes)
@@ -62,7 +65,8 @@
     if ((rc = dev_alloc(ix, &p, b))) return rc;
     d.enc = (const uint32_t*)p;
     ix->bufs.push_back({p, b});
-    b = (d.nkmers + 16) * 4;
+    d.slot_colours = H.slot_colours;
+    b = (d.nkmers + 16 + (H.slot_colours ? kr::kSlotColourDict : 0u)) * 4;
     if ((rc = dev_alloc(ix, &p, b))) return rc;
     d.se = (const uint32_t*)p;
     ix->bufs.push_back({p, b});
@@ -291,7 +295,7 @@
     const kr_lib_view& lv = v->libs[i];
     if (lv.r >= v->m) return kr::fail(KR_ERR_FORMAT, "library residue r >= m");
     if (lv.nnodes != v->tree_nnodes + 1) return kr::fail(KR_ERR_FORMAT, "crecord nnodes does not match the tree");
-    L[i] = DescLib{lv.nkmers, 0, lv.nrows, lv.nsubsets, lv.nnodes, lv.frac ? lv.r + 1 : 1u};
+    L[i] = DescLib{lv.nkmers, 0, lv.nrows, lv.nsubsets, lv.nnodes, lv.frac ? lv.r + 1 : 1u, 0, 0, 0};
     if (lv.frac)
       for (uint32_t q = 0; q <= lv.r; ++q) res_lib[q] = (int32_t)i;
     else
@@ -329,6 +333,7 @@
       const uint32_t w = (uint32_t)atoi(e);
       H.slot_log2w = (fits32 && w >= 5 && w <= 9) ? w : 0u;
     }
+    H.slot_colours = (H.slot_log2w >= 5u && H.slot_log2w <= 8u && !(getenv("KR_SLOT_COLOURS") && atoi(getenv("KR_SLOT_COLOURS")) == 0)) ? 1u : 0u;
   }
   std::vector<std::vector<uint2>> hpse(v->nlibs);
   std::vector<std::vector<uint32_t>> cls(v->nlibs), lists(v->nlibs);
@@ -375,7 +380,7 @@
       src_inc = t_inc.get();
     }
     HIP_TRY(hipMemset((void*)d.enc, 0xFF, (d.nkmers + 16) * 4));
-    HIP_TRY(hipMemset((void*)d.se, 0, (d.nkmers + 16) * 4));
+    HIP_TRY(hipMemset((void*)d.se, 0, (d.nkmers + 16 + (H.slot_colours ? kr::kSlotColourDict : 0u)) * 4));
     if (lv.nsubsets > kColMask) return kr::fail(KR_ERR_ARG, "kr_index_upload: more than 2^30 colours is not supported");
     DevBuf<uint32_t> b_cls;
     if (!b_cls.reserve((uint64_t)lv.nsubsets + 4)) return alloc_failed("kr_index_upload: staging");
@@ -389,8 +394,41 @@
     if (lv.nrows && H.slot_log2w == kSlotFilter) {
       hipLaunchKernelGGL(kr_build_fslots, dim3(8192), dim3(256), 0, 0, d.bkt, d.enc, lv.nrows, (uint4*)d.slots);
       hipLaunchKernelGGL(kr_build_sx, dim3(8192), dim3(256), 0, 0, d.bkt, d.enc, d.se, lv.nrows, (uint2*)d.sx);
-    } else if (lv.nrows && H.slot_log2w)
-      hipLaunchKernelGGL(kr_build_slots, dim3(8192), dim3(256), 0, 0, d.bkt, d.enc, lv.nrows, slot_words(H.slot_log2w), (uint32_t*)d.slots);
+    } else if (lv.nrows && H.slot_log2w) {
+      DevBuf<uint32_t> b_cnt, b_val;
+      DevBuf<uint16_t> b_code;
+      DevBuf<unsigned long long> b_ncoded;
+      const uint32_t nkeys = H.nleaves + lv.nsubsets;
+      if (H.slot_colours) {
+        if (!b_cnt.reserve((uint64_t)nkeys + 1) || !b_val.reserve((uint64_t)nkeys + 1) || !b_code.reserve((uint64_t)nkeys + 1) || !b_ncoded.reserve(1))
+          return alloc_failed("kr_index_upload: staging");
+        HIP_TRY(hipMemset(b_cnt.get(), 0, ((uint64_t)nkeys + 1) * 4));
+        HIP_TRY(hipMemset(b_val.get(), 0, ((uint64_t)nkeys + 1) * 4));
+        HIP_TRY(hipMemset(b_ncoded.get(), 0, 8));
+        if (lv.nkmers) hipLaunchKernelGGL(kr_colour_hist, dim3(512), dim3(1024), 0, 0, d.se, lv.nkmers, H.nleaves, nkeys, b_cnt.get(), b_val.get());
+        std::vector<uint32_t> cnt(nkeys), val(nkeys), dict;
+        if (nkeys) {
+          HIP_TRY(hipMemcpy(cnt.data(), b_cnt.get(), (uint64_t)nkeys * 4, hipMemcpyDeviceToHost));
+          HIP_TRY(hipMemcpy(val.data(), b_val.get(), (uint64_t)nkeys * 4, hipMemcpyDeviceToHost));
+        }
+        uint32_t limit = kr::kSlotNoCode;
+        if (const char* e = getenv("KR_SLOT_COLOUR_DICT")) limit = std::min<uint32_t>(limit, (uint32_t)std::max(0, atoi(e)));
+        const std::vector<uint32_t> order = kr::slot_colour_ranking(cnt.data(), nkeys, limit);
+        std::vector<uint16_t> code_of((size_t)nkeys + 1, (uint16_t)kr::kSlotNoCode);
+        dict.assign(kr::kSlotColourDict, 0u);
+        for (size_t c = 0; c < order.size(); ++c) code_of[order[c]] = (uint16_t)c, dict[c] = val[order[c]];
+        HIP_TRY(hipMemcpy(b_code.get(), code_of.data(), code_of.size() * 2, hipMemcpyHostToDevice));
+        HIP_TRY(hipMemcpy((void*)(d.se + d.nkmers + 16), dict.data(), dict.size() * 4, hipMemcpyHostToDevice));
+        L[i].ndict = (uint32_t)order.size();
+      }
+      hipLaunchKernelGGL(kr_build_slots, dim3(8192), dim3(256), 0, 0, d.bkt, d.enc, lv.nrows, slot_words(H.slot_log2w), (uint32_t*)d.slots, d.se,
+                         H.slot_colours ? b_code.get() : nullptr, H.nleaves, nkeys, H.slot_colours ? b_ncoded.get() : nullptr);
+      if (H.slot_colours) {
+        unsigned long long nc = 0;
+        HIP_TRY(hipMemcpy(&nc, b_ncoded.get(), 8, hipMemcpyDeviceToHost));
+        L[i].ncoded = nc;
+      }
+    }
     HIP_TRY(hipDeviceSynchronize());
     t_cmer.reset(), t_inc.reset(), b_cls.reset();
     if (lv.nsubsets) HIP_TRY(hipMemcpy((void*)d.pse, hpse[i].data(), (uint64_t)lv.nsubsets * 8, hipMemcpyHostToDevice));
@@ -403,6 +441,7 @@
     return kr::fail(KR_ERR_FORMAT, "inc-* is not monotone or a bucket exceeds 2^24 entries / 2^40 offset");
   }
   HIP_TRY(hipMemcpy((void*)ix->dix.res_lib, res_lib.data(), (uint64_t)v->m * 4, hipMemcpyHostToDevice));
+  memcpy(ix->desc.data() + sizeof(H), L.data(), L.size() * sizeof(DescLib));
   *out = ix.release();
   return KR_OK;
 }
@@ -420,6 +459,33 @@
 uint64_t kr_index_device_bytes(const kr_index* ix) { return ix ? ix->bytes : 0; }
 uint32_t kr_index_slot_words(const kr_index* ix) { return ix && ix->slot_log2w ? slot_words(ix->slot_log2w) : 0; }
 uint32_t kr_index_slot_format(const kr_index* ix) { return ix ? ix->slot_log2w : 0; }
+int kr_index_slot_colour_stats(const kr_index* ix, uint64_t* dict_codes, uint64_t* coded_entries, uint64_t* total_entries)
+{
+  if (!ix || ix->desc.size() < sizeof(DescHeader)) return kr::fail(KR_ERR_ARG, "kr_index_slot_colour_stats: null argument");
+  DescHeader H;
+  memcpy(&H, ix->desc.data(), sizeof(H));
+  uint64_t nd = 0, nc = 0, nt = 0;
+  for (uint32_t i = 0; i < H.nlibs; ++i) {
+    DescLib l;
+    memcpy(&l, ix->desc.data() + sizeof(H) + (size_t)i * sizeof(DescLib), sizeof(l));
+    nd += l.ndict, nc += l.ncoded, nt += l.nkmers;
+  }
+  if (dict_codes) *dict_codes = H.slot_colours ? nd : 0;
+  if (coded_entries) *coded_entries = H.slot_colours ? nc : 0;
+  if (total_entries) *total_entries = nt;
+  return KR_OK;
+}
+int kr_debug_slot_colour_layout(uint32_t n, uint32_t words, const uint32_t* counts, uint32_t nkeys, uint32_t limit, uint32_t* ncol, uint32_t* order,
+                                uint32_t* norder)
+{
+  if (ncol) *ncol = kr::slot_ncol(n, words);
+  if (counts && order && norder) {
+    const std::vector<uint32_t> o = kr::slot_colour_ranking(counts, nkeys, limit);
+    if (!o.empty()) memcpy(order, o.data(), o.size() * 4);
+    *norder = (uint32_t)o.size();
+  }
+  return KR_OK;
+}
 
 int kr_index_export(const kr_index* ix, void* desc, uint64_t* desc_bytes, kr_index_buffer* bufs, uint32_t* nbufs)
 {
diff --git a/krepp_amd/csrc/kr_host_stream.inc b/krepp_amd/csrc/kr_host_stream.inc
--- a/krepp_amd/csrc/kr_host_stream.inc
+++ b/krepp_amd/csrc/kr_host_stream.inc
@@ -387,7 +387,8 @@
   BatchOut& o = L.out;
   const dim3 block(kScanWaves * kWave);
   auto grid = [&](uint32_t blocks) { return dim3(std::min<uint32_t>((L.nreads + kScanWaves - 1) / kScanWaves, blocks)); };
-  static const bool pipe = !getenv("KR_SCAN_PIPE") || atoi(getenv("KR_SCAN_PIPE")) != 0;
+  const char* pipe_env = getenv("KR_SCAN_PIPE");
+  const bool pipe = !pipe_env || atoi(pipe_env) != 0;
   with_bools([&](auto SL, auto TAP) {
     if (s->fk) {
       hipLaunchKernelGGL((kr_scan_filt_kernel_t<KR_SCAN_FILT_DEPTH, KR_SCAN_FILT_WPE, SL.value, TAP.value>), grid(s->scan_filt_blocks), block, 0, st, dix, s->dp, L.in, o);
@@ -1018,7 +1019,7 @@
   CounterCombine how;
 };
 constexpr CounterRule kCounterRules[] = {
-  {kCtErr, kOr}, {kCtL2Reads, kSum}, {kCtTapHits, kSum}, {kCtRecords, kSum},
+  {kCtErr, kOr}, {kCtL2Reads, kSum}, {kCtTapHits, kSum}, {kCtTapCoded, kSum}, {kCtRecords, kSum},
   {kCtStEvents, kSum}, {kCtStKeys, kSum}, {kCtStBatches, kSum}, {kCtStBig, kSum}, {kCtStLevelTiles, kSum}, {kCtStMaxKeys, kMax}, {kCtStMaxEvents, kMax},
   {kCtCycLevel, kSum}, {kCtCycFinalize, kSum}, {kCtCycRead, kSum},
   {kCtProblems, kSum}, {kCtStackSpills, kSum}, {kCtTileHoles, kSum},
@@ -1370,6 +1371,13 @@
   return KR_OK;
 }
 
+int kr_debug_tap_coded_items(kr_stream* s, uint64_t* coded)
+{
+  if (!s || !coded || !s->waited) return kr::fail(KR_ERR_STATE, "kr_debug_tap_coded_items: collect a KR_TAP_HITS batch first");
+  *coded = s->h_counters[kCtTapCoded];
+  return KR_OK;
+}
+
 int kr_batch_readtaps(kr_stream* s, const kr_readtap** taps)
 {
   if (!s || !taps || !s->waited) return kr::fail(KR_ERR_STATE, "kr_batch_readtaps: collect a batch first");
```

Measured after the change: 126.1 million reads/s (median of 6 runs). No clear change (+0.9%).
